# DerrickXuNu/CoBEVT

Hardware: AMD Instinct MI355X
Metric: bev_frames_per_sec (higher is better)
Workload: dtype bf16

## Files before the change

cobevt_amd/csrc/elementwise.hip:

```cpp
#include "warp_common.hpp"
#include "wave_ops.hpp"

namespace cobevt {

template <typename T>
__global__ __launch_bounds__(256) void layernorm_kernel(const T* in, const float* gamma, const float* beta, T* out,
                                                        int rows, int C, float eps, int navg, long avg_stride,
                                                        long in_batch_stride, int rows_per_batch) {
    const int G = C >> 3;
    const int gid = (blockIdx.x * 256 + threadIdx.x) / G;
    const int gl = threadIdx.x & (G - 1);
    if (gid >= rows) return;
    const int bb = gid / rows_per_batch, rr = gid - bb * rows_per_batch;
    const T* src = in + (size_t)bb * in_batch_stride + (size_t)rr * C + gl * 8;
    float v[8];
    load8<T>(src, v);
    if (navg > 1) {
        for (int s = 1; s < navg; ++s) {
            float w[8];
            load8<T>(src + (size_t)s * avg_stride, w);
#pragma unroll
            for (int e = 0; e < 8; ++e) v[e] += w[e];
        }
        const float inv = 1.0f / (float)navg;
#pragma unroll
        for (int e = 0; e < 8; ++e) v[e] *= inv;
    }
    float s = 0.f;
#pragma unroll
    for (int e = 0; e < 8; ++e) s += v[e];
    s = wave_sum_xor(s, G);
    const float mean = s / (float)C;
    float q = 0.f;
#pragma unroll
    for (int e = 0; e < 8; ++e) { const float d = v[e] - mean; q += d * d; }
    q = wave_sum_xor(q, G);
    const float rstd = rsqrtf(q / (float)C + eps);
#pragma unroll
    for (int e = 0; e < 8; ++e) {
        v[e] = (v[e] - mean) * rstd;
        if (gamma) v[e] = v[e] * gamma[gl * 8 + e] + beta[gl * 8 + e];
    }
    store8<T>(out + (size_t)gid * C + gl * 8, v);
}

constexpr int kEmbedPixPerBlock = 256;
constexpr int kRayPixPerBlock = 64;

template <typename T>
__global__ __launch_bounds__(256) void ray_embed_kernel(const float* I_inv, const float* E_inv, const float* plane,
                                                        const float* w_img, const float* w_cam, T* out, int BN,
                                                        int hw, int D) {
    const int G = D >> 3;
    const int gl = threadIdx.x & (G - 1), gp = threadIdx.x / G, ngroups = 256 / G;
    const int bn = blockIdx.y;
    const float* I = I_inv + bn * 9;
    const float* E = E_inv + bn * 16;
    float wi[8][4], ce[8];
#pragma unroll
    for (int e = 0; e < 8; ++e) {
        const int ch = gl * 8 + e;
        const float4 a = *(const float4*)(w_img + ch * 4), c = *(const float4*)(w_cam + ch * 4);
        wi[e][0] = a.x; wi[e][1] = a.y; wi[e][2] = a.z; wi[e][3] = a.w;
        ce[e] = c.x * E[3] + c.y * E[7] + c.z * E[11] + c.w * E[15];
    }
    const int p0 = blockIdx.x * kRayPixPerBlock;
    constexpr int U = 4;
    for (int pb = p0 + gp; pb < min(p0 + kRayPixPerBlock, hw); pb += ngroups * U) {
        float pxs[U], pys[U], pzs[U];
#pragma unroll
        for (int u = 0; u < U; ++u) {
            const int q = min(pb + u * ngroups, hw - 1);
            pxs[u] = plane[q]; pys[u] = plane[hw + q]; pzs[u] = plane[2 * hw + q];
        }
#pragma unroll
        for (int u = 0; u < U; ++u) {
        const int pix = pb + u * ngroups;
        if (pix >= min(p0 + kRayPixPerBlock, hw)) break;
        const float px = pxs[u], py = pys[u], pz = pzs[u];
        float cam[4];
#pragma unroll
        for (int r = 0; r < 3; ++r) cam[r] = I[r * 3 + 0] * px + I[r * 3 + 1] * py + I[r * 3 + 2] * pz;
        cam[3] = 1.f;
        float d4[4];
#pragma unroll
        for (int r = 0; r < 4; ++r)
            d4[r] = E[r * 4 + 0] * cam[0] + E[r * 4 + 1] * cam[1] + E[r * 4 + 2] * cam[2] + E[r * 4 + 3] * cam[3];
        float v[8], ss = 0.f;
#pragma unroll
        for (int e = 0; e < 8; ++e) {
            const float de = wi[e][0] * d4[0] + wi[e][1] * d4[1] + wi[e][2] * d4[2] + wi[e][3] * d4[3];
            v[e] = de - ce[e];
            ss += v[e] * v[e];
        }
        ss = wave_sum_xor(ss, G);
        const float inv = 1.0f / (sqrtf(ss) + 1e-7f);
#pragma unroll
        for (int e = 0; e < 8; ++e) v[e] *= inv;
        store8<T>(out + ((size_t)bn * hw + pix) * D + gl * 8, v);
        }
    }
}

template <typename T>
__global__ __launch_bounds__(256) void bev_embed_kernel(const float* E_inv, const float* world, const float* w_bev,
                                                        const float* b_bev, const float* w_cam, const T* x, T* out,
                                                        int B, int n, int hw, int D, int x_bcast) {
    const int G = D >> 3;
    const int gl = threadIdx.x & (G - 1), gp = threadIdx.x / G, ngroups = 256 / G;
    const int bn = blockIdx.y, b = x_bcast ? 0 : bn / n;
    const float* E = E_inv + bn * 16;
    float wb[8][2], off[8];
#pragma unroll
    for (int e = 0; e < 8; ++e) {
        const int ch = gl * 8 + e;
        const float4 c = *(const float4*)(w_cam + ch * 4);
        wb[e][0] = w_bev[ch * 2 + 0]; wb[e][1] = w_bev[ch * 2 + 1];
        off[e] = c.x * E[3] + c.y * E[7] + c.z * E[11] + c.w * E[15];
    }
    float bb[8];
#pragma unroll
    for (int e = 0; e < 8; ++e) bb[e] = b_bev[gl * 8 + e];
    const int p0 = blockIdx.x * kEmbedPixPerBlock;
    constexpr int U = 4;
    for (int pb = p0 + gp; pb < min(p0 + kEmbedPixPerBlock, hw); pb += ngroups * U) {
        float wxs[U], wys[U], xvs[U][8];
#pragma unroll
        for (int u = 0; u < U; ++u) {
            const int q = min(pb + u * ngroups, hw - 1);
            wxs[u] = world[q]; wys[u] = world[hw + q];
            load8<T>(x + ((size_t)b * hw + q) * D + gl * 8, xvs[u]);
        }
#pragma unroll
        for (int u = 0; u < U; ++u) {
        const int pix = pb + u * ngroups;
        if (pix >= min(p0 + kEmbedPixPerBlock, hw)) break;
        const float wx = wxs[u], wy = wys[u];
        float v[8], ss = 0.f;
#pragma unroll
        for (int e = 0; e < 8; ++e) {
            const float we = wb[e][0] * wx + wb[e][1] * wy + bb[e];
            v[e] = we - off[e];
            ss += v[e] * v[e];
        }
        ss = wave_sum_xor(ss, G);
        const float inv = 1.0f / (sqrtf(ss) + 1e-7f);
#pragma unroll
        for (int e = 0; e < 8; ++e) v[e] = v[e] * inv + xvs[u][e];
        store8<T>(out + ((size_t)bn * hw + pix) * D + gl * 8, v);
        }
    }
}

template <typename T>
__global__ __launch_bounds__(256) void agent_max_kernel(const T* in, T* out, int B, int L, long per8) {
    const long gid = (long)blockIdx.x * 256 + threadIdx.x;
    if (gid >= (long)B * per8) return;
    const long b = gid / per8, i = gid - b * per8;
    float m[8];
    load8<T>(in + ((size_t)b * L * per8 + i) * 8, m);
    for (int l = 1; l < L; ++l) {
        float v[8];
        load8<T>(in + (((size_t)b * L + l) * per8 + i) * 8, v);
#pragma unroll
        for (int e = 0; e < 8; ++e) m[e] = fmaxf(m[e], v[e]);
    }
    store8<T>(out + (size_t)gid * 8, m);
}

template <typename T>
__global__ __launch_bounds__(256) void maxpool3x3s2_kernel(const T* in, T* out, int N, int H, int W, int C, int Ho,
                                                           int Wo) {
    const int G = C >> 3;
    const long gid = ((long)blockIdx.x * 256 + threadIdx.x) / G;
    const int gl = threadIdx.x & (G - 1);
    if (gid >= (long)N * Ho * Wo) return;
    const int n = (int)(gid / (Ho * Wo)), rem = (int)(gid - (long)n * Ho * Wo);
    const int oh = rem / Wo, ow = rem - oh * Wo;
    float m[8];
#pragma unroll
    for (int e = 0; e < 8; ++e) m[e] = -INFINITY;
    for (int kh = 0; kh < 3; ++kh) {
        const int ih = oh * 2 - 1 + kh;
        if (ih < 0 || ih >= H) continue;
        for (int kw = 0; kw < 3; ++kw) {
            const int iw = ow * 2 - 1 + kw;
            if (iw < 0 || iw >= W) continue;
            float v[8];
            load8<T>(in + (((size_t)n * H + ih) * W + iw) * C + gl * 8, v);
#pragma unroll
            for (int e = 0; e < 8; ++e) m[e] = fmaxf(m[e], v[e]);
        }
    }
    store8<T>(out + gid * C + gl * 8, m);
}

template <typename TI, typename TO>
__global__ __launch_bounds__(256) void to_nhwc_kernel(const TI* in, TO* out, int N, int C, int H, int W, long sN, long sC,
                                                      long sH, long sW) {
    const long i = (long)blockIdx.x * 256 + threadIdx.x;
    const long total = (long)N * C * H * W;
    if (i >= total) return;
    const int c = (int)(i % C);
    long r = i / C;
    const int w = (int)(r % W); r /= W;
    const int h = (int)(r % H);
    const int n = (int)(r / H);
    store_elem<TO>(out, i, load_elem<TI>(in, n * sN + c * sC + h * sH + w * sW));
}
template <typename TI, typename TO>
__global__ __launch_bounds__(256) void from_nhwc_kernel(const TI* in, TO* out, int N, int C, int H, int W, long sN,
                                                        long sC, long sH, long sW) {
    const long i = (long)blockIdx.x * 256 + threadIdx.x;
    const long total = (long)N * C * H * W;
    if (i >= total) return;
    const int c = (int)(i % C);
    long r = i / C;
    const int w = (int)(r % W); r /= W;
    const int h = (int)(r % H);
    const int n = (int)(r / H);
    store_elem<TO>(out, n * sN + c * sC + h * sH + w * sW, load_elem<TI>(in, i));
}

template <typename T>
__global__ __launch_bounds__(256) void regroup_kernel(const T* in, const int* record_len, T* out, float* mask, int B,
                                                      int max_cav, long chunks_per_agent) {
    const long i = (long)blockIdx.x * 256 + threadIdx.x;
    const long total = (long)B * max_cav * chunks_per_agent;
    if (i >= total) return;
    const long agent_slot = i / chunks_per_agent, within = i - agent_slot * chunks_per_agent;
    const int b = (int)(agent_slot / max_cav), l = (int)(agent_slot - (long)b * max_cav);
    int off = 0;
    for (int bb = 0; bb < b; ++bb) off += record_len[bb];
    const bool present = l < record_len[b];
    uint4 v = make_uint4(0, 0, 0, 0);
    if (present) v = ((const uint4*)in)[(long)(off + l) * chunks_per_agent + within];
    ((uint4*)out)[i] = v;
    if (within == 0) mask[agent_slot] = present ? 1.f : 0.f;
}

template <typename T>
__global__ __launch_bounds__(256) void sttf_warp_kernel(const T* x, const float* tmat, const float* cav_mask, T* out,
                                                        float* com_mask, const int* record_len, float* cav_out,
                                                        int B, int Lc, int H, int W, int C,
                                                        float discrete_ratio, float downsample_rate) {
    const int G = C >> 3;
    const int bl = blockIdx.y;
    const int b = bl / Lc, l = bl - b * Lc;
    __shared__ Affine th_feat, th_mask;
// ... 315 lines not shown
```

cobevt_amd/csrc/proj_chain128.hip:

```cpp
#include "row_chain.hpp"
#include "wave_ops.hpp"

namespace cobevt {

namespace {

constexpr int kFp = 0, kFn = 32, kMaxNnt = 8;
constexpr int kTab = (kFn + kMaxNnt * 8) * 1024;
constexpr int kSc = 0, kSh = 128, kBp = 256, kBn = 384;
constexpr int kTabFloats = 640;
constexpr int kLdsBytes = kTab + kTabFloats * 4;

template <int NNT, int NW>
__global__ __launch_bounds__(NW * 64, 1) void proj_chain128_kernel(RowChainParams p, int nblk) {
    extern __shared__ __attribute__((aligned(16))) unsigned char smem[];
    const uint4* wl = (const uint4*)smem;
    float* tab = (float*)(smem + kTab);
    const int tid = threadIdx.x, lane = tid & 63, wave = tid >> 6;
    const int h = lane >> 5, ql = lane & 31;

    {
        uint4* dst = (uint4*)smem;
        constexpr int TOTAL = (kFn + NNT * 8) * 64, PER = (TOTAL + NW * 64 - 1) / (NW * 64);
        uint4 tmp[PER];
#pragma unroll
        for (int u = 0; u < PER; ++u) {
            const int i = tid + u * NW * 64, ic = i < TOTAL ? i : TOTAL - 1;
            const int f = ic >> 6, ln = ic & 63, hh = ln >> 5, q = ln & 31;
            const uint4* base = f < kFn ? p.wp + (size_t)f * 64 : p.wn + (size_t)(f - kFn) * 64;
            const unsigned char* a0 = (const unsigned char*)(base + (f < kFn ? ln : q)) + (f < kFn ? 0 : 8 * hh);
            const unsigned char* a1 = f < kFn ? a0 + 8 : (const unsigned char*)(base + 32 + q) + 8 * hh;
            const uint2 lo = *(const uint2*)a0, hi = *(const uint2*)a1;
            tmp[u] = make_uint4(lo.x, lo.y, hi.x, hi.y);
        }
#pragma unroll
        for (int u = 0; u < PER; ++u) {
            const int i = tid + u * NW * 64;
            if (i < TOTAL) dst[i] = tmp[u];
        }
        for (int i = tid; i < kTabFloats; i += NW * 64) {
            float v;
            if (i < kSh) v = p.pre_scale ? p.pre_scale[i] : 1.f;
            else if (i < kBp) v = p.pre_shift ? p.pre_shift[i - kSh] : 0.f;
            else if (i < kBn) v = p.bp ? p.bp[i - kBp] : 0.f;
            else v = (p.bn && i - kBn < p.Nn) ? p.bn[i - kBn] : 0.f;
            tab[i] = v;
        }
    }
    __syncthreads();

    int opq = 0;
    const float relu_floor = (p.pre_scale && p.pre_relu) ? 0.f : -INFINITY;
    auto load_tile = [&](uint4 (&fr)[8], int first) {
#pragma unroll
        for (int g = 0; g < 8; ++g) fr[g] = wl[(first + g) * 64 + lane + opq];
    };
    const int nwaves = gridDim.x * NW;
    for (int blk = blockIdx.x * NW + wave; blk < nblk; blk += nwaves) {
        asm volatile("" : "+v"(opq));
        const int m0 = blk * 32;
        const bool live = m0 + ql < p.M;
        const size_t grow = live ? m0 + ql : p.M - 1;
        const bf16_t* arow = p.a + grow * 128;
        uint4 af[8], sk[8];
#pragma unroll
        for (int g = 0; g < 8; ++g) af[g] = *(const uint4*)(arow + 16 * g + 8 * h);
        if (p.skip) {
            const bf16_t* srow = p.skip + (size_t)(grow % p.skip_rows) * 128;
#pragma unroll
            for (int g = 0; g < 8; ++g) sk[g] = *(const uint4*)(srow + 16 * g + 8 * h);
        } else {
#pragma unroll
            for (int g = 0; g < 8; ++g) sk[g] = make_uint4(0, 0, 0, 0);
        }
#pragma unroll
        for (int g = 0; g < 8; ++g) {
            float v[8];
            chunk_to_f32<bf16_t>(af[g], v);
            const float* sc = tab + kSc + 16 * g + 8 * h + opq;
            const float4 s0 = *(const float4*)sc, s1 = *(const float4*)(sc + 4);
            const float4 t0 = *(const float4*)(sc + (kSh - kSc)), t1 = *(const float4*)(sc + (kSh - kSc) + 4);
            v[0] = fmaxf(fmaf(v[0], s0.x, t0.x), relu_floor); v[1] = fmaxf(fmaf(v[1], s0.y, t0.y), relu_floor);
            v[2] = fmaxf(fmaf(v[2], s0.z, t0.z), relu_floor); v[3] = fmaxf(fmaf(v[3], s0.w, t0.w), relu_floor);
            v[4] = fmaxf(fmaf(v[4], s1.x, t1.x), relu_floor); v[5] = fmaxf(fmaf(v[5], s1.y, t1.y), relu_floor);
            v[6] = fmaxf(fmaf(v[6], s1.z, t1.z), relu_floor); v[7] = fmaxf(fmaf(v[7], s1.w, t1.w), relu_floor);
            af[g] = f32_to_chunk<bf16_t>(v);
        }

        float y[4][16];
        uint4 fr[2][8];
        load_tile(fr[0], kFp);
#pragma unroll
        for (int t = 0; t < 4; ++t) {
            f32x16 acc;
#pragma unroll
            for (int r = 0; r < 16; ++r) acc[r] = 0.f;
            load_tile(fr[(t + 1) & 1], t < 3 ? kFp + (t + 1) * 8 : kFn);
            __builtin_amdgcn_sched_barrier(0);
#pragma unroll
            for (int g = 0; g < 8; ++g) mfma_kgroup<bf16_t>(fr[t & 1][g], af[g], acc);
#pragma unroll
            for (int m = 0; m < 2; ++m) {
                uint2 s0 = make_uint2(sk[2 * t + m].x, sk[2 * t + m].y), s1 = make_uint2(sk[2 * t + m].z, sk[2 * t + m].w);
                half_swap(s0, s1);
                const float4 b0 = *(const float4*)(tab + kBp + 32 * t + 16 * m + 4 * h + opq);
                const float4 b1 = *(const float4*)(tab + kBp + 32 * t + 16 * m + 8 + 4 * h + opq);
                float* d = &y[t][8 * m];
                d[0] = rbf(acc[8 * m + 0] + b0.x + bf2f(s0.x & 0xffff)); d[1] = rbf(acc[8 * m + 1] + b0.y + bf2f(s0.x >> 16));
                d[2] = rbf(acc[8 * m + 2] + b0.z + bf2f(s0.y & 0xffff)); d[3] = rbf(acc[8 * m + 3] + b0.w + bf2f(s0.y >> 16));
                d[4] = rbf(acc[8 * m + 4] + b1.x + bf2f(s1.x & 0xffff)); d[5] = rbf(acc[8 * m + 5] + b1.y + bf2f(s1.x >> 16));
                d[6] = rbf(acc[8 * m + 6] + b1.z + bf2f(s1.y & 0xffff)); d[7] = rbf(acc[8 * m + 7] + b1.w + bf2f(s1.y >> 16));
            }
        }
        if (p.out) {
            bf16_t* orow = p.out + grow * 128;
#pragma unroll
            for (int i = 0; i < 8; ++i) {
                const uint4 pk = pack8(&y[i >> 1][8 * (i & 1)]);
                uint2 r0 = make_uint2(pk.x, pk.y), r1 = make_uint2(pk.z, pk.w);
                half_swap(r0, r1);
                if (live) *(uint4*)(orow + 16 * i + 8 * h) = make_uint4(r0.x, r0.y, r1.x, r1.y);
            }
        }
        if (p.next_ln) {
            float s = 0.f;
#pragma unroll
            for (int t = 0; t < 4; ++t)
#pragma unroll
                for (int r = 0; r < 16; ++r) s += y[t][r];
            const float mean = xhalf_sum(s) * (1.0f / 128.0f);
            float q = 0.f;
#pragma unroll
            for (int t = 0; t < 4; ++t)
#pragma unroll
                for (int r = 0; r < 16; ++r) { const float d = y[t][r] - mean; q += d * d; }
            const float rstd = rsqrtf(xhalf_sum(q) * (1.0f / 128.0f) + p.eps_next);
#pragma unroll
            for (int t = 0; t < 4; ++t)
#pragma unroll
                for (int r = 0; r < 16; ++r) y[t][r] = (y[t][r] - mean) * rstd;
        }
        uint4 yh[8];
#pragma unroll
        for (int t = 0; t < 4; ++t)
#pragma unroll
            for (int u = 0; u < 2; ++u) yh[2 * t + u] = pack8(&y[t][8 * u]);

        bf16_t* nrow = p.out_next + grow * p.Nn;
#pragma unroll
        for (int n = 0; n < NNT; ++n) {
            f32x16 acc;
#pragma unroll
            for (int r = 0; r < 16; ++r) acc[r] = 0.f;
            if (n + 1 < NNT) load_tile(fr[(n + 1) & 1], kFn + (n + 1) * 8);
            __builtin_amdgcn_sched_barrier(0);
#pragma unroll
            for (int g = 0; g < 8; ++g) mfma_kgroup<bf16_t>(fr[n & 1][g], yh[g], acc);
            float nv[16];
#pragma unroll
            for (int k = 0; k < 4; ++k) {
                const float4 b = *(const float4*)(tab + kBn + 32 * n + 8 * k + 4 * h + opq);
                nv[4 * k] = acc[4 * k] + b.x; nv[4 * k + 1] = acc[4 * k + 1] + b.y;
                nv[4 * k + 2] = acc[4 * k + 2] + b.z; nv[4 * k + 3] = acc[4 * k + 3] + b.w;
            }
#pragma unroll
            for (int m = 0; m < 2; ++m) {
                const uint4 pk = pack8(&nv[8 * m]);
                uint2 r0 = make_uint2(pk.x, pk.y), r1 = make_uint2(pk.z, pk.w);
                half_swap(r0, r1);
                if (live) *(uint4*)(nrow + 32 * n + 16 * m + 8 * h) = make_uint4(r0.x, r0.y, r1.x, r1.y);
            }
        }
    }
}

template <int NNT> int launch128(const RowChainParams& p, hipStream_t stream) {
    constexpr int NW = 8;
    cobevt::allow_dynamic_lds<proj_chain128_kernel<NNT, NW>>(kLdsBytes);
    const int nblk = (p.M + 31) / 32;
    int blocks = (nblk + NW - 1) / NW;
    if (blocks > 256) blocks = 256;
    hipLaunchKernelGGL((proj_chain128_kernel<NNT, NW>), dim3((unsigned)blocks), dim3(NW * 64), kLdsBytes, stream, p, nblk);
    return cobevt::launch_status();
}

}

int launch_proj_chain128(const RowChainParams& p, hipStream_t stream) {
    if (p.C != 128 || !p.wn || !p.out_next || p.Nn % 32 != 0 || p.Nn > 32 * kMaxNnt || p.next_act != 0) return -1;
    if (p.M < 32768) return -1;
    switch (p.Nn / 32) {
        case 4: return launch128<4>(p, stream);
        case 8: return launch128<8>(p, stream);
        default: return -1;
    }
}

}
```

cobevt_amd/csrc/row_chain.hip:

```cpp
#include "row_chain.hpp"
#include "wave_ops.hpp"

namespace cobevt {

constexpr int kRcRow = 256 + 16;
constexpr int kRcHRow = 512 + 16;
template <int ROWS> struct RcLds {
    static constexpr int A = 0;
    static constexpr int Y = A + ROWS * kRcRow;
    static constexpr int H = Y + ROWS * kRcRow;
    static constexpr int TOTAL = H + ROWS * kRcHRow;
    static constexpr int BIAS = TOTAL;
    static constexpr int BYTES = TOTAL + 4 * 1536;
};
constexpr int kRcBp = 0, kRcB1 = 128, kRcB2 = 384, kRcPg = 512, kRcPb = 640, kRcBn = 768, kRcBnMax = 768, kRcBiasFloats = 1536;

__device__ __forceinline__ void rc_normalise(float (&v)[16], int sub, int C, float eps) {
    float s = 0.f;
#pragma unroll
    for (int e = 0; e < 16; ++e) s += v[e];
    s = lane8_sum(s);
    const float mean = s / (float)C;
    float q = 0.f;
#pragma unroll
    for (int e = 0; e < 16; ++e) { const float d = (sub * 16 + e) < C ? v[e] - mean : 0.f; q += d * d; }
    q = lane8_sum(q);
    const float rstd = rsqrtf(q / (float)C + eps);
#pragma unroll
    for (int e = 0; e < 16; ++e) v[e] = (sub * 16 + e) < C ? (v[e] - mean) * rstd : 0.f;
}

template <int NPASS, int ROWS, bool FULL, bool MLP = true>
__global__ __launch_bounds__(ROWS * 8, 4) void row_chain_kernel(RowChainParams p) {
    extern __shared__ __attribute__((aligned(16))) unsigned char smem[];
    unsigned char* As = smem + RcLds<ROWS>::A;
    unsigned char* Ys = smem + RcLds<ROWS>::Y;
    unsigned char* Hs = smem + RcLds<ROWS>::H;

    const int tid = threadIdx.x, lane = tid & 63, wave = tid >> 6;
    const int h = lane >> 5, ql = lane & 31;
    const int wm = wave >> 2, wn = wave & 3;
    const int m0 = blockIdx.x * ROWS;
    const int ngc = FULL ? 8 : (p.C * 2 + 31) / 32;
    const int row = wm * 32 + ql;
    const bool row_ok = m0 + row < p.M;

    auto load_frags = [&](uint4 (&b)[8], const uint4* w, int tile, int nkg, int kg0, int n) {
        const uint4* src = w + ((size_t)tile * nkg + kg0) * 64 + lane;
#pragma unroll
        for (int g = 0; g < 8; ++g)
            if (g < n) b[g] = src[g * 64];
        __builtin_amdgcn_sched_barrier(0);
    };
    f32x16 acc;
    auto mma = [&](const unsigned char* A, int a_off, const uint4 (&b)[8], int n, bool zero) {
        if (zero) {
#pragma unroll
            for (int r = 0; r < 16; ++r) acc[r] = 0.f;
        }
#pragma unroll
        for (int g = 0; g < 8; ++g)
            if (g < n) {
                const uint4 af = *(const uint4*)(A + a_off + g * 32);
                mfma_kgroup<bf16_t>(b[g], af, acc);
            }
    };
    const int cbase = wn * 32 + 4 * h;
    const float* sb = (const float*)(smem + RcLds<ROWS>::BIAS);
    {
        float* w = (float*)(smem + RcLds<ROWS>::BIAS);
        constexpr int NT = ROWS * 8, NIT = kRcBiasFloats / NT;
        static_assert(kRcBiasFloats % NT == 0, "bias table fill");
        float val[NIT];
        bool keep[NIT];
#pragma unroll
        for (int it = 0; it < NIT; ++it) {
            const int i = tid + it * NT;
            const float* src = i < kRcB1 ? p.bp : i < kRcB2 ? p.b1 : i < kRcPg ? p.b2 : i < kRcPb ? p.post_g : i < kRcBn ? p.post_b : p.bn;
            const int j = i < kRcB1 ? i : i < kRcB2 ? i - kRcB1 : i < kRcPg ? i - kRcB2 : i < kRcPb ? i - kRcPg : i < kRcBn ? i - kRcPb : i - kRcBn;
            const int n = i < kRcB1 ? p.C : i < kRcB2 ? p.Hd : i < kRcBn ? p.C : p.Nn;
            keep[it] = (src != nullptr) & (j < n);
            val[it] = (src ? src : p.b1)[keep[it] ? j : 0];
        }
#pragma unroll
        for (int it = 0; it < NIT; ++it) w[tid + it * NT] = keep[it] ? val[it] : 0.f;
    }
    auto bias4 = [&](int table, int col0) { return *(const float4*)(sb + table + col0); };
    auto pack4 = [&](float x, float y, float z, float w) { return make_uint2(pack_bf2(x, y), pack_bf2(z, w)); };

    uint4 fa[8], fb[8];
    const int abase = row * kRcRow + h * 16;

    load_frags(fa, p.wp, wn, 8, 0, ngc);
    {
        const int r = tid >> 3, sub = tid & 7;
        const bool ok = m0 + r < p.M;
#pragma unroll
        for (int j = 0; j < 2; ++j) {
            const int k = (sub * 2 + j) * 8;
            uint4 v = make_uint4(0, 0, 0, 0);
            if (ok && k < p.C) v = *(const uint4*)(p.a + (size_t)(m0 + r) * p.C + k);
            if (!MLP && p.pre_scale) {
                float f[8];
                chunk_to_f32<bf16_t>(v, f);
                const float4 s0 = *(const float4*)(p.pre_scale + k), s1 = *(const float4*)(p.pre_scale + k + 4);
                const float4 t0 = *(const float4*)(p.pre_shift + k), t1 = *(const float4*)(p.pre_shift + k + 4);
                const float sc[8] = {s0.x, s0.y, s0.z, s0.w, s1.x, s1.y, s1.z, s1.w}, sh[8] = {t0.x, t0.y, t0.z, t0.w, t1.x, t1.y, t1.z, t1.w};
#pragma unroll
                for (int e = 0; e < 8; ++e) {
                    f[e] = fmaf(f[e], sc[e], sh[e]);
                    if (p.pre_relu) f[e] = fmaxf(f[e], 0.f);
                }
                v = ok ? f32_to_chunk<bf16_t>(f) : make_uint4(0, 0, 0, 0);
            }
            *(uint4*)(As + r * kRcRow + (sub * 2 + j) * 16) = v;
        }
    }
    uint2 skp[4];
#pragma unroll
    for (int k = 0; k < 4; ++k) {
        const int col0 = cbase + 8 * k;
        skp[k] = make_uint2(0, 0);
        if (p.skip && row_ok && col0 < p.C) skp[k] = *(const uint2*)(p.skip + (size_t)((m0 + row) % p.skip_rows) * p.C + col0);
    }
    __syncthreads();

    mma(As, abase, fa, ngc, true);
    if (MLP) load_frags(fb, p.w1, wn, 8, 0, ngc);
    else load_frags(fb, p.wn, wn, 8, 0, ngc);
#pragma unroll
    for (int k = 0; k < 4; ++k) {
        const int col0 = cbase + 8 * k;
        const float4 b = bias4(kRcBp, col0);
        float v0 = acc[4 * k] + b.x + bf2f(skp[k].x & 0xffff), v1 = acc[4 * k + 1] + b.y + bf2f(skp[k].x >> 16);
        float v2 = acc[4 * k + 2] + b.z + bf2f(skp[k].y & 0xffff), v3 = acc[4 * k + 3] + b.w + bf2f(skp[k].y >> 16);
        if (col0 >= p.C) v0 = v1 = v2 = v3 = 0.f;
        *(uint2*)(Ys + row * kRcRow + col0 * 2) = pack4(v0, v1, v2, v3);
    }
    __syncthreads();
    float* stage = (float*)Hs;
    constexpr int SROW = kRcHRow / 4;
    if constexpr (MLP) {

    if (NPASS == 2) load_frags(fa, p.w1, 4 + wn, 8, 0, ngc);
    else load_frags(fa, p.w2, wn, p.Hdp / 16, 0, 8);
    {
        const int r = tid >> 3, sub = tid & 7;
        float v[16];
        chunk_to_f32<bf16_t>(*(const uint4*)(Ys + r * kRcRow + sub * 32), v);
        chunk_to_f32<bf16_t>(*(const uint4*)(Ys + r * kRcRow + sub * 32 + 16), v + 8);
        rc_normalise(v, sub, p.C, p.eps1);
        *(uint4*)(As + r * kRcRow + sub * 32) = f32_to_chunk<bf16_t>(v);
// ... 34 lines not shown
    __syncthreads();
#pragma unroll
    for (int k = 0; k < 4; ++k) {
        const int col0 = cbase + 8 * k;
        const float4 b = bias4(kRcB2, col0);
        const uint2 y = *(const uint2*)(Ys + row * kRcRow + col0 * 2);
        float4 z = make_float4(0.f, 0.f, 0.f, 0.f);
        if (col0 < p.C)
            z = make_float4(acc[4 * k] + b.x + bf2f(y.x & 0xffff), acc[4 * k + 1] + b.y + bf2f(y.x >> 16),
                            acc[4 * k + 2] + b.z + bf2f(y.y & 0xffff), acc[4 * k + 3] + b.w + bf2f(y.y >> 16));
        *(float4*)(stage + row * SROW + col0) = z;
    }
    } else {
#pragma unroll
        for (int k = 0; k < 4; ++k) {
            const int col0 = cbase + 8 * k;
            const uint2 y = *(const uint2*)(Ys + row * kRcRow + col0 * 2);
            *(float4*)(stage + row * SROW + col0) = make_float4(bf2f(y.x & 0xffff), bf2f(y.x >> 16), bf2f(y.y & 0xffff), bf2f(y.y >> 16));
        }
    }
    const int npn = p.wn ? (p.Nn + 127) / 128 : 0;
    __syncthreads();

    {
        const int r = tid >> 3, sub = tid & 7;
        const bool live = m0 + r < p.M;
        float v[16];
#pragma unroll
        for (int e = 0; e < 16; e += 4) {
            const float4 t = *(const float4*)(stage + r * SROW + sub * 16 + e);
            v[e] = t.x; v[e + 1] = t.y; v[e + 2] = t.z; v[e + 3] = t.w;
        }
        if (p.post_g) {
            rc_normalise(v, sub, p.C, p.eps_post);
#pragma unroll
            for (int e = 0; e < 16; e += 4) {
                const float4 g = *(const float4*)(sb + kRcPg + sub * 16 + e), b = *(const float4*)(sb + kRcPb + sub * 16 + e);
                v[e] = v[e] * g.x + b.x; v[e + 1] = v[e + 1] * g.y + b.y;
                v[e + 2] = v[e + 2] * g.z + b.z; v[e + 3] = v[e + 3] * g.w + b.w;
            }
        }
        uint4 o[2];
        o[0] = f32_to_chunk<bf16_t>(v);
        o[1] = f32_to_chunk<bf16_t>(v + 8);
        if (live && (MLP || p.out)) {
#pragma unroll
            for (int j = 0; j < 2; ++j) {
                const int c0 = sub * 16 + j * 8;
                if (c0 < p.C) *(uint4*)(p.out + (size_t)(m0 + r) * p.C + c0) = o[j];
            }
        }
        if (!npn) return;

        if (p.next_ln) {
            chunk_to_f32<bf16_t>(o[0], v);
            chunk_to_f32<bf16_t>(o[1], v + 8);
            rc_normalise(v, sub, p.C, p.eps_next);
            o[0] = f32_to_chunk<bf16_t>(v);
            o[1] = f32_to_chunk<bf16_t>(v + 8);
        }
        *(uint4*)(As + r * kRcRow + sub * 32) = o[0];
        *(uint4*)(As + r * kRcRow + sub * 32 + 16) = o[1];
    }
    __syncthreads();
    auto next_pass = [&](int pass, const uint4 (&cur)[8], uint4 (&nxt)[8]) {
        if (pass + 1 < npn) load_frags(nxt, p.wn, (pass + 1) * 4 + wn, 8, 0, ngc);
        mma(As, abase, cur, ngc, true);
#pragma unroll
        for (int k = 0; k < 4; ++k) {
            const int col0 = pass * 128 + cbase + 8 * k;
            const float4 b = bias4(kRcBn, col0);
            float v0 = acc[4 * k] + b.x, v1 = acc[4 * k + 1] + b.y, v2 = acc[4 * k + 2] + b.z, v3 = acc[4 * k + 3] + b.w;
            if (p.next_act == 1) { v0 = fmaxf(v0, 0.f); v1 = fmaxf(v1, 0.f); v2 = fmaxf(v2, 0.f); v3 = fmaxf(v3, 0.f); }
            else if (p.next_act == 2) { v0 = gelu_bf16(v0); v1 = gelu_bf16(v1); v2 = gelu_bf16(v2); v3 = gelu_bf16(v3); }
            *(uint2*)(Ys + row * kRcRow + (cbase + 8 * k) * 2) = pack4(v0, v1, v2, v3);
        }
        __syncthreads();
        {
            const int r = tid >> 3, sub = tid & 7;
            if (m0 + r < p.M) {
#pragma unroll
                for (int j = 0; j < 2; ++j) {
                    const int c0 = pass * 128 + sub * 16 + j * 8;
                    if (c0 < p.Nn) *(uint4*)(p.out_next + (size_t)(m0 + r) * p.Nn + c0) = *(const uint4*)(Ys + r * kRcRow + sub * 32 + j * 16);
                }
            }
        }
        if (pass + 1 < npn) __syncthreads();
    };
    for (int pass = 0; pass < npn; pass += 2) {
        next_pass(pass, fb, fa);
        if (pass + 1 < npn) next_pass(pass + 1, fa, fb);
    }
}

template <int NPASS, int ROWS, bool FULL, bool MLP = true>
static void launch_chain(const RowChainParams& p, hipStream_t stream) {
    cobevt::allow_dynamic_lds<row_chain_kernel<NPASS, ROWS, FULL, MLP>>(RcLds<ROWS>::BYTES);
    const unsigned blocks = (unsigned)((p.M + ROWS - 1) / ROWS);
    hipLaunchKernelGGL((row_chain_kernel<NPASS, ROWS, FULL, MLP>), dim3(blocks), dim3(ROWS * 8), RcLds<ROWS>::BYTES, stream, p);
}

}

using namespace cobevt;

extern "C" int cobevt_attn_mlp_chain(const void* a, const void* skip, void* out, const void* wp, const float* bp,
                                     const void* w1, const float* b1, const void* w2, const float* b2,
                                     const float* post_gamma, const float* post_beta, const void* wnext, const float* bnext,
                                     void* out_next, const int* dims, float eps1, float eps_post, float eps_next,
                                     hipStream_t stream) {
    if (!a || !out || !wp || !w1 || !b1 || !w2 || !b2 || !dims) return COBEVT_ERR_ARG;
    if (dims[0] != 0 && dims[0] != 1) return COBEVT_ERR_ARG;
    if (dims[0] == 1) {
        if ((post_gamma == nullptr) != (post_beta == nullptr) || (wnext == nullptr) != (out_next == nullptr)) return COBEVT_ERR_ARG;
        const int M = dims[1], sr = dims[9] > 0 ? dims[9] : dims[1];
        if (M < 1 || sr > M || M % sr || (wnext && (dims[7] < 0 || dims[7] > 2))) return COBEVT_ERR_SHAPE;
        const int rc = launch_row_chain_f32(a, skip, out, wp, bp, w1, b1, w2, b2, post_gamma, post_beta, wnext, bnext, out_next, M, dims[2], dims[3],
                                            dims[4], dims[5], dims[6], dims[7], sr, eps1, eps_post, eps_next, stream);
        return rc < 0 ? COBEVT_ERR_UNSUPPORTED : rc;
    }
    RowChainParams p;
    p.a = (const bf16_t*)a; p.skip = (const bf16_t*)skip; p.out = (bf16_t*)out;
    p.wp = (const uint4*)wp; p.bp = bp; p.w1 = (const uint4*)w1; p.b1 = b1; p.w2 = (const uint4*)w2; p.b2 = b2;
    p.post_g = post_gamma; p.post_b = post_beta;
    p.wn = (const uint4*)wnext; p.bn = bnext; p.out_next = (bf16_t*)out_next;
    p.M = dims[1]; p.C = dims[2]; p.Hd = dims[3]; p.Hdp = dims[4];
    p.Nn = dims[5]; p.next_ln = dims[6]; p.next_act = dims[7];
    p.skip_rows = dims[9] > 0 ? dims[9] : p.M;
    p.eps1 = eps1; p.eps_post = eps_post; p.eps_next = eps_next;
    p.pre_scale = p.pre_shift = nullptr; p.pre_relu = 0;
    if (p.M < 1 || p.C < 8 || p.C > 128 || p.C % 8 || p.Hd < 8 || p.Hd > 256 || p.Hd % 8) return COBEVT_ERR_SHAPE;
    if (p.Hdp % 128 || p.Hdp < p.Hd || p.Hdp > 256) return COBEVT_ERR_SHAPE;
    if (p.skip_rows > p.M || p.M % p.skip_rows) return COBEVT_ERR_SHAPE;
    if ((post_gamma == nullptr) != (post_beta == nullptr)) return COBEVT_ERR_ARG;
    if ((wnext == nullptr) != (out_next == nullptr)) return COBEVT_ERR_ARG;
    if (wnext && (p.Nn < 8 || p.Nn % 8 || p.Nn > kRcBnMax || p.next_act < 0 || p.next_act > 2)) return COBEVT_ERR_SHAPE;
    if (dims[8] == 0) {
        const int rc = launch_row_chain64(p, stream);
        if (rc >= 0) return rc;
    }
    const int rows = dims[8] == 64 ? 64 : 32;
    const bool two = p.Hd > 128, full = p.C == 128;
    if (rows == 64) {
        if (two) { if (full) launch_chain<2, 64, true>(p, stream); else launch_chain<2, 64, false>(p, stream); }
        else { if (full) launch_chain<1, 64, true>(p, stream); else launch_chain<1, 64, false>(p, stream); }
    } else {
        if (two) { if (full) launch_chain<2, 32, true>(p, stream); else launch_chain<2, 32, false>(p, stream); }
        else { if (full) launch_chain<1, 32, true>(p, stream); else launch_chain<1, 32, false>(p, stream); }
    }
    return cobevt::launch_status();
}

extern "C" int cobevt_proj_chain(const void* a, const float* pre_scale, const float* pre_shift, const void* skip, const void* wp,
                                 const float* bp, void* out, const void* wnext, const float* bnext, void* out_next, const int* dims,
                                 float eps_next, hipStream_t stream) {
    if (!a || !wp || !wnext || !bnext || !out_next || !dims) return COBEVT_ERR_ARG;
    if ((pre_scale == nullptr) != (pre_shift == nullptr)) return COBEVT_ERR_ARG;
    if (dims[0] != 0) return COBEVT_ERR_UNSUPPORTED;
    RowChainParams p;
    p.a = (const bf16_t*)a; p.skip = (const bf16_t*)skip; p.out = (bf16_t*)out;
    p.wp = (const uint4*)wp; p.bp = bp;
    p.w1 = (const uint4*)wnext; p.b1 = bnext; p.w2 = (const uint4*)wnext; p.b2 = bnext;
    p.post_g = p.post_b = nullptr;
    p.wn = (const uint4*)wnext; p.bn = bnext; p.out_next = (bf16_t*)out_next;
    p.M = dims[1]; p.C = dims[2]; p.Hd = 8; p.Hdp = 128;
    p.Nn = dims[3]; p.next_ln = dims[4]; p.next_act = dims[5];
    p.skip_rows = dims[6] > 0 ? dims[6] : p.M;
    p.pre_scale = pre_scale; p.pre_shift = pre_shift; p.pre_relu = dims[7];
    p.eps1 = 0.f; p.eps_post = 0.f; p.eps_next = eps_next;
    if (p.M < 1 || p.C != 128) return COBEVT_ERR_SHAPE;
    if (p.Nn < 8 || p.Nn % 8 || p.Nn > kRcBnMax || p.next_act < 0 || p.next_act > 2) return COBEVT_ERR_SHAPE;
    if (p.skip_rows > p.M || p.M % p.skip_rows) return COBEVT_ERR_SHAPE;
    if (dims[8] == 0) {
        const int rc = launch_proj_chain128(p, stream);
        if (rc >= 0) return rc;
    }
    launch_chain<1, 32, true, false>(p, stream);
    return cobevt::launch_status();
}
```

cobevt_amd/csrc/row_chain.hpp:

```cpp
#pragma once
#include "common.hpp"

namespace cobevt {

struct RowChainParams {
    const bf16_t* a;
    const bf16_t* skip;
    bf16_t* out;
    const uint4* wp;
    const float* bp;
    const uint4* w1;
    const float* b1;
    const uint4* w2;
    const float* b2;
    const float* post_g;
    const float* post_b;
    const uint4* wn;
    const float* bn;
    bf16_t* out_next;
    int M, C, Hd, Hdp;
    int Nn, next_ln, next_act, skip_rows;
    float eps1, eps_post, eps_next;
    const float* pre_scale;
    const float* pre_shift;
    int pre_relu;
};

int launch_row_chain64(const RowChainParams& p, hipStream_t stream);
int launch_proj_chain128(const RowChainParams& p, hipStream_t stream);

int launch_row_chain_f32(const void* a, const void* skip, void* out, const void* wp, const float* bp, const void* w1, const float* b1,
                         const void* w2, const float* b2, const float* post_g, const float* post_b, const void* wnext, const float* bnext,
                         void* out_next, int M, int C, int Hd, int Hdp, int Nn, int next_ln, int next_act, int skip_rows, float eps1,
                         float eps_post, float eps_next, hipStream_t stream);

}
```

cobevt_amd/host/fax_modules.py:

```python
import torch
import torch.nn as nn

from .. import ops
from ..lib import CobevtHipError
from . import runtime as rt
from . import training
from .runtime import HipModule


def generate_grid(height, width):
    xs = torch.linspace(0, 1, width)
    ys = torch.linspace(0, 1, height)
    gx = xs[None, :].expand(height, width)
    gy = ys[:, None].expand(height, width)
    return torch.stack([gx, gy, torch.ones(height, width)], 0)[None].contiguous()


def get_view_matrix(h=200, w=200, h_meters=100.0, w_meters=100.0, offset=0.0):
    sh = h / h_meters
    sw = w / w_meters
    return [[0., -sw, w / 2.], [-sh, 0., h * offset + h / 2.], [0., 0., 1.]]


class Bottleneck(HipModule):
# ... 72 lines not shown
        self.heads = dim // dim_head
        self.scale = dim_head ** -0.5
        self.window_size = window_size
        self.to_qkv = nn.Linear(dim, dim * 3, bias=False)
        self.attend = nn.Sequential(nn.Softmax(dim=-1), nn.Dropout(dropout))
        self.to_out = nn.Sequential(nn.Linear(dim, dim, bias=False), nn.Dropout(dropout))
        self.rel_pos_bias = nn.Embedding((2 * window_size - 1) ** 2, self.heads)
        pos = torch.arange(window_size)
        gi, gj = torch.meshgrid(pos, pos, indexing="ij")
        grid = torch.stack([gi.reshape(-1), gj.reshape(-1)], -1)
        rel_pos = grid[:, None, :] - grid[None, :, :] + window_size - 1
        rel_pos_indices = (rel_pos * torch.tensor([2 * window_size - 1, 1])).sum(dim=-1)
        self.register_buffer("rel_pos_indices", rel_pos_indices, persistent=False)

    def forward_nhwc(self, x, out=None):
        b, h, w, d = x.shape
        if h != self.window_size or w != self.window_size:
            raise CobevtHipError("FAX global attention expects a %dx%d map" % (self.window_size, self.window_size))
        qkv = ops.linear(x, rt.linear_plan(self, "qkv", self.to_qkv))
        a = torch.empty((b, h, w, d), device=x.device, dtype=x.dtype)
        m = ops.tokmap(0, 1, h, w, h, w)
        table = rt.f32_param(self, "bias", self.rel_pos_bias.weight)
        ops.window_attention(qkv, qkv, qkv, a, m, m, m, b, self.heads, self.scale, 3 * d, 3 * d, 3 * d, d, koff=d,
                             voff=2 * d, bias_table=table, bias_L=1)
        return ops.linear(a, rt.linear_plan(self, "out", self.to_out[0]), out=out)

    def forward(self, x):
        if self.training:
            return training.global_attention(self, x)
        self._require_inference(x)
        return rt.like_input(rt.nchw_view(self.forward_nhwc(rt.to_nhwc(x))), x)


class CrossWinAttention(HipModule):

    def __init__(self, dim, heads, dim_head, qkv_bias, rel_pos_emb=False, norm=nn.LayerNorm):
        super().__init__()
        if dim_head != 32:
            raise CobevtHipError("the HIP attention kernel is built for dim_head = 32")
        self.scale = dim_head ** -0.5
        self.heads = heads
        self.dim_head = dim_head
        self.rel_pos_emb = rel_pos_emb
        self.to_q = nn.Sequential(norm(dim), nn.Linear(dim, heads * dim_head, bias=qkv_bias))
        self.to_k = nn.Sequential(norm(dim), nn.Linear(dim, heads * dim_head, bias=qkv_bias))
        self.to_v = nn.Sequential(norm(dim), nn.Linear(dim, heads * dim_head, bias=qkv_bias))
        self.proj = nn.Linear(heads * dim_head, dim)

    def add_rel_pos_emb(self, x):
        return x

    def _project(self, name, seq, x, out=None):
        return ops.linear(x, rt.linear_plan(self, name, seq[1], ln=seq[0]), out=out)

    def project_kv(self, k_src, v_src, out_k=None, out_v=None):
        return self._project("k", self.to_k, k_src, out_k), self._project("v", self.to_v, v_src, out_v)

    def q_plan(self):
        return rt.linear_plan(self, "q", self.to_q[1], ln=self.to_q[0])

    def attend_projected(self, q_src, kt, vt, qmap, kmap, omap, batch, out_shape, qt=None, ldkv=None, kvoff=0):
        inner = self.heads * self.dim_head
        if qt is None:
            qt = self._project("q", self.to_q, q_src)
        ld = inner if ldkv is None else ldkv
        a = torch.empty(tuple(out_shape) + (inner,), device=qt.device, dtype=qt.dtype)
        ops.window_attention(qt, kt, vt, a, qmap, kmap, omap, batch, self.heads, self.scale, inner, ld, ld, inner,
                             koff=kvoff, voff=kvoff, mean_q=qmap[1] > 1)
        return a

    def attend_core(self, q_src, k_src, v_src, qmap, kmap, omap, batch, out_shape):
        kt, vt = self.project_kv(k_src, v_src)
        return self.attend_projected(q_src, kt, vt, qmap, kmap, omap, batch, out_shape)

    def attend(self, q_src, k_src, v_src, qmap, kmap, omap, batch, skip, out_shape):
        a = self.attend_core(q_src, k_src, v_src, qmap, kmap, omap, batch, out_shape)
        return ops.linear(a, rt.linear_plan(self, "proj", self.proj), residual=skip)

    def forward(self, q, k, v, skip=None):
        if self.training:
            return training.cross_win_attention(self, q, k, v, skip)
        self._require_inference(q, k, v, skip)
        assert k.shape == v.shape
        b, n, X, Y, W1, W2, _ = q.shape
        _, nk, kx, ky, w1, w2, _ = k.shape
        assert X * Y == kx * ky
        qmap = (2, n, X * W1, Y * W2, W1, W2, X, Y)
        kmap = (2, nk, kx * w1, ky * w2, w1, w2, kx, ky)
        omap = (2, 1, X * W1, Y * W2, W1, W2, X, Y)
        sk = rt.as_compute(skip) if skip is not None else None
        z = self.attend(rt.as_compute(q), rt.as_compute(k), rt.as_compute(v), qmap, kmap, omap, b, sk,
                        (b, X, Y, W1, W2))
        return rt.like_input(z, q)


class CrossViewSwapAttention(HipModule):

    def __init__(self, feat_height, feat_width, feat_dim, dim, index, image_height, image_width, qkv_bias, q_win_size,
                 feat_win_size, heads, dim_head, bev_embedding_flag, rel_pos_emb=False, no_image_features=False,
                 skip=True, norm=nn.LayerNorm):
        super().__init__()
        image_plane = generate_grid(feat_height, feat_width)[None]
        image_plane[:, :, 0] *= image_width
        image_plane[:, :, 1] *= image_height
        self.register_buffer("image_plane", image_plane, persistent=False)
        self.feature_linear = nn.Sequential(nn.BatchNorm2d(feat_dim), nn.ReLU(), nn.Conv2d(feat_dim, dim, 1, bias=False))
        if no_image_features:
            self.feature_proj = None
        else:
            self.feature_proj = nn.Sequential(nn.BatchNorm2d(feat_dim), nn.ReLU(), nn.Conv2d(feat_dim, dim, 1, bias=False))
        self.bev_embed_flag = bev_embedding_flag[index]
        if self.bev_embed_flag:
            self.bev_embed = nn.Conv2d(2, dim, 1)
        self.img_embed = nn.Conv2d(4, dim, 1, bias=False)
        self.cam_embed = nn.Conv2d(4, dim, 1, bias=False)
        self.q_win_size = q_win_size[index]
        self.feat_win_size = feat_win_size[index]
        self.rel_pos_emb = rel_pos_emb
        self.cross_win_attend_1 = CrossWinAttention(dim, heads[index], dim_head[index], qkv_bias)
        self.cross_win_attend_2 = CrossWinAttention(dim, heads[index], dim_head[index], qkv_bias)
        self.skip = skip
        self.prenorm_1 = norm(dim)
        self.prenorm_2 = norm(dim)
        self.mlp_1 = nn.Sequential(nn.Linear(dim, 2 * dim), nn.GELU(), nn.Linear(2 * dim, dim))
        self.mlp_2 = nn.Sequential(nn.Linear(dim, 2 * dim), nn.GELU(), nn.Linear(2 * dim, dim))
        self.postnorm = norm(dim)
        self.dim = dim

    def _padded_hw(self, h, w):
        wh, ww = self.feat_win_size
        hp = ((h + wh) // wh) * wh if h % wh != 0 else h
        wp = ((w + ww) // ww) * ww if w % ww != 0 else w
        return hp, wp

    def _proj_mlp(self, name, attn, a, skip, prenorm, mlp, postnorm=None, next_plan=None):
        post = None
        if postnorm is not None:
            post = (rt.f32_param(self, name + ".post.w", postnorm.weight), rt.f32_param(self, name + ".post.b", postnorm.bias),
                    postnorm.eps)
        return ops.attn_mlp_chain(a, skip, rt.linear_plan(attn, "proj", attn.proj),
                                  rt.linear_plan(self, name + ".0", mlp[0], act=2, ln=prenorm),
                                  rt.linear_plan(self, name + ".2", mlp[2]), post, next_plan=next_plan)

    def prepare_kv(self, feature, I_inv, E_inv, batch, out=None):
        bn, h, w, _ = feature.shape
        d, dt = self.dim, feature.dtype
        n = bn // batch
        w1, w2 = self.feat_win_size
        hp, wp = self._padded_hw(h, w)
        padded = (hp, wp) != (h, w)
        plane = rt.f32_param(self, "plane", self.image_plane, (3, h * w))
        w_img = rt.f32_param(self, "w_img", self.img_embed.weight, (d, 4))
        w_cam = rt.f32_param(self, "w_cam", self.cam_embed.weight, (d, 4))
        img = ops.ray_embed(I_inv, E_inv, plane, w_img, w_cam, h * w, d, dt).reshape(bn, h, w, d)

        def kv_buffer(tag):
            if not padded:
                return None
            return self._plan("kvpad.%s.%dx%dx%d" % (tag, bn, hp, wp), [self.img_embed.weight],
                              lambda dt_, dev: torch.zeros((bn, hp, wp, d), device=feature.device, dtype=dt))

        o = out if out is not None else {}
        pk, pv = self._pair_plan("k"), self._pair_plan("v")
        plan_key = rt.conv_plan(self, "fproj", self.feature_proj[2], pre_bn=self.feature_proj[0]) if self.feature_proj is not None else None
        plan_val = rt.conv_plan(self, "flin", self.feature_linear[2], pre_bn=self.feature_linear[0])
        if (not padded and plan_key is not None and ops.proj_chain_fusable(feature, plan_key, pk, img)
                and ops.proj_chain_fusable(feature, plan_val, pv, None)):
            kk = ops.proj_chain(feature, plan_key, pk, residual=img, out_next=o.get("kk"))
            vv = ops.proj_chain(feature, plan_val, pv, out_next=o.get("vv"))
            return {"n": n, "hp": hp, "wp": wp, "kk": kk, "vv": vv}
        if not padded and plan_key is not None and ops.proj_chain_kv_fusable(feature, plan_key, plan_val, pk, pv, img):
            kk, vv = ops.proj_chain_kv(feature, plan_key, plan_val, pk, pv, residual=img, out_k=o.get("kk"), out_v=o.get("vv"))
            return {"n": n, "hp": hp, "wp": wp, "kk": kk, "vv": vv}
        if self.feature_proj is not None:
            key = ops.conv2d(feature, plan_key, residual=img, out=kv_buffer("key"))
        elif padded:
            key = ops.copy_into_interior(img, kv_buffer("key"))
        else:
            key = img
        val = ops.conv2d(feature, plan_val, out=kv_buffer("val"))
        kk = ops.linear(key, pk, out=o.get("kk"))
        vv = ops.linear(val, pv, out=o.get("vv"))
        return {"n": n, "hp": hp, "wp": wp, "kk": kk, "vv": vv}

    def _pair_plan(self, which):
        a1, a2 = getattr(self.cross_win_attend_1, "to_" + which), getattr(self.cross_win_attend_2, "to_" + which)
        if a1[0].eps != a2[0].eps:
            raise CobevtHipError("the two cross attentions normalise their keys / values with different eps")

        def build(dt, dev):
            ws, bs = [], []
            for ln, lin in ((a1[0], a1[1]), (a2[0], a2[1])):
                w = lin.weight.detach().double().cpu()
                b = lin.bias.detach().double().cpu() if lin.bias is not None else torch.zeros(w.shape[0], dtype=torch.float64)
                g, be = ln.weight.detach().double().cpu(), ln.bias.detach().double().cpu()
                bs.append(b + w @ be)
                ws.append(w * g[None, :])
            return ops.ConvPlan(torch.cat(ws), torch.cat(bs), dtype=dt, device=dev, ln_folded_eps=a1[0].eps)
        return self._plan("pair_" + which, rt.module_tensors(a1[0], a1[1], a2[0], a2[1]), build)

    def forward_query(self, index, x, bev, E_inv, kv, next_plan=None):
        b, H, W, d = x.shape
        n, hp, wp = kv["n"], kv["hp"], kv["wp"]
        W1, W2 = self.q_win_size
        w1, w2 = self.feat_win_size
        if self.bev_embed_flag:
            grid = getattr(bev, "grid%d" % index)
            world = rt.f32_param(self, "world%d" % index, grid[:2], (2, H * W))
            w_bev = rt.f32_param(self, "w_bev", self.bev_embed.weight, (d, 2))
            b_bev = rt.f32_param(self, "b_bev", self.bev_embed.bias)
            w_cam = rt.f32_param(self, "w_cam", self.cam_embed.weight, (d, 4))
            q1 = ops.bev_embed_linear(E_inv, world, w_bev, b_bev, w_cam, x.reshape(b, H * W, d), n,
                                      self.cross_win_attend_1.q_plan())
            query, nq = None, n
        else:
            x = x.contiguous()
            query, nq, q1 = x, 1, None
        qmap_n = ops.tokmap(0, nq, H, W, W1, W2)
        qmap_1 = ops.tokmap(0, 1, H, W, W1, W2)
        kwin = ops.tokmap(0, n, hp, wp, w1, w2)
        kgrid = ops.tokmap(1, n, hp, wp, w1, w2)
        if qmap_1[6] * qmap_1[7] != kwin[6] * kwin[7]:
            raise CobevtHipError("query windows %dx%d != key windows %dx%d" % (qmap_1[6], qmap_1[7], kwin[6], kwin[7]))
        inner = self.cross_win_attend_1.heads * self.cross_win_attend_1.dim_head
        a = self.cross_win_attend_1.attend_projected(query, kv["kk"], kv["vv"], qmap_n, kwin, qmap_1, b, (b, H, W), qt=q1,
                                                     ldkv=2 * inner, kvoff=0)
        y, q2 = self._proj_mlp("mlp1", self.cross_win_attend_1, a, x if self.skip else None, self.prenorm_1, self.mlp_1,
                               next_plan=self.cross_win_attend_2.q_plan())
        a = self.cross_win_attend_2.attend_projected(y, kv["kk"], kv["vv"], qmap_1, kgrid, qmap_1, b, (b, H, W), qt=q2,
                                                     ldkv=2 * inner, kvoff=inner)
        return self._proj_mlp("mlp2", self.cross_win_attend_2, a, y if self.skip else None, self.prenorm_2, self.mlp_2,
                              self.postnorm, next_plan=next_plan)

    def forward_nhwc(self, index, x, bev, feature, I_inv, E_inv):
        return self.forward_query(index, x, bev, E_inv, self.prepare_kv(feature, I_inv, E_inv, x.shape[0]))

    def forward(self, index, x, bev, feature, I_inv, E_inv):
        if self.training:
            return training.cross_view_swap_attention(self, index, x, bev, feature, I_inv, E_inv)
        self._require_inference(x, feature, I_inv, E_inv)
        b, n = feature.shape[:2]
        f = rt.to_nhwc(feature.reshape(b * n, *feature.shape[2:]))
        Ii = I_inv.reshape(b * n, 3, 3).to(torch.float32).contiguous()
        Ei = E_inv.reshape(b * n, 4, 4).to(torch.float32).contiguous()
        y = self.forward_nhwc(index, rt.to_nhwc(x), bev, f, Ii, Ei)
        return rt.like_input(rt.nchw_view(y), x)


class _Downsample(HipModule):

    def __init__(self, dim_in, dim_mid, dim_out):
        super().__init__()
        mods = [nn.Conv2d(dim_in, dim_mid, kernel_size=3, stride=1, padding=1, bias=False), nn.PixelUnshuffle(2),
                nn.Conv2d(dim_out, dim_out, 3, padding=1, bias=False), nn.BatchNorm2d(dim_out), nn.ReLU(inplace=True),
                nn.Conv2d(dim_out, dim_out, 1, padding=0, bias=False), nn.BatchNorm2d(dim_out)]
        for i, m in enumerate(mods):
            self.add_module(str(i), m)

    def __getitem__(self, i):
        return getattr(self, str(i))

    def forward_nhwc(self, x, out=None):
        y = ops.conv2d(x, rt.conv_plan(self, "c0", self[0], store_mode=1))
        y = ops.conv2d(y, rt.conv_plan(self, "c2", self[2], self[3], act=1))
        return ops.conv2d(y, rt.conv_plan(self, "c5", self[5], self[6]), out=out)


class FAXModule(HipModule):

    _downsample_div = 4

    def __init__(self, config):
        super().__init__()
        middle = config["middle"]
        dim = config["dim"]
        self.backbone_output_shape = config["backbone_output_shape"]
        assert len(middle) == len(self.backbone_output_shape)
        cross_view = config["cross_view"]
        cross_view_swap = config["cross_view_swap"]
        cross_views, layers, downsample_layers = [], [], []
        for i, (feat_shape, num_layers) in enumerate(zip(self.backbone_output_shape, middle)):
            _, _, _, feat_dim, feat_height, feat_width = tuple(feat_shape)
            cross_views.append(CrossViewSwapAttention(feat_height, feat_width, feat_dim, dim[i], i, **cross_view,
                                                      **cross_view_swap))
            layers.append(nn.Sequential(*[ResNetBottleNeck(dim[i]) for _ in range(num_layers)]))
            if i < len(middle) - 1:
                downsample_layers.append(nn.Sequential(_Downsample(dim[i], dim[i] // self._downsample_div, dim[i + 1])))
        self.bev_embedding = BEVEmbedding(dim[0], **config["bev_embedding"])
        self.cross_views = nn.ModuleList(cross_views)
        self.layers = nn.ModuleList(layers)
        self.downsample_layers = nn.ModuleList(downsample_layers)
        self.self_attn = Attention(dim[-1], **config["self_attn"])

    taps = None

    def forward_features(self, features, I_inv, E_inv, batch, kv=None, levels=None, x=None, out=None):
        nlev = len(self.cross_views)
        first, last = (0, nlev) if levels is None else levels
        if first == 0:
            dt = rt.get_compute_dtype()
            prior = self._plan("prior", [self.bev_embedding.learned_features],
                               lambda d_, dev: self.bev_embedding.learned_features.detach().permute(1, 2, 0).to(dt).contiguous())
            x = prior[None].expand(batch, *prior.shape)
        for i, (cross_view, feature, layer) in enumerate(zip(self.cross_views, features, self.layers)):
            if i < first or i >= last:
                continue
            kvi = kv[i]() if kv is not None else cross_view.prepare_kv(feature, I_inv, E_inv, batch)
            blocks = list(layer)
            y1 = None
            if blocks and not (x.dtype == torch.bfloat16 and ops.USE_BOTTLENECK and x.shape[-1] == 128
                               and blocks[0].conv1.weight.shape[:2] == (32, 128)):
                x, y1 = cross_view.forward_query(i, x, self.bev_embedding, E_inv, kvi, next_plan=blocks[0].entry_plan())
            else:
                x = cross_view.forward_query(i, x, self.bev_embedding, E_inv, kvi)
            for j, blk in enumerate(blocks):
                x = blk.forward_nhwc(x, y1=y1 if j == 0 else None)
            if self.taps is not None:
                self.taps["level%d" % i] = x
# ... 27 lines not shown
```

cobevt_amd/lib.py:

```python
import ctypes
import os

import torch

_HERE = os.path.dirname(os.path.abspath(__file__))
LIB_PATH = os.path.join(_HERE, "csrc", "libcobevt_hip.so")
LIB_PATH = os.environ.get("COBEVT_HIP_LIB") or LIB_PATH

_c_int_p = ctypes.POINTER(ctypes.c_int)
_c_long_p = ctypes.POINTER(ctypes.c_long)
_c_float_p = ctypes.POINTER(ctypes.c_float)
_vp = ctypes.c_void_p

SIGNATURES = {
    "cobevt_abi_version": (ctypes.c_int, []),
    "cobevt_strerror": (ctypes.c_char_p, [ctypes.c_int]),
    "cobevt_conv2d_nhwc": (ctypes.c_int, [_vp, _vp, _vp, _vp, _vp, _vp, _vp, _vp, _c_int_p, _vp]),
    "cobevt_conv3x3_nhwc": (ctypes.c_int, [_vp, _vp, _vp, _vp, _vp, _c_int_p, _vp]),
    "cobevt_basicblock_nhwc": (ctypes.c_int, [_vp, _vp, _vp, _vp, _vp, _vp, _c_int_p, _vp]),
    "cobevt_dsblock_nhwc": (ctypes.c_int, [_vp, _vp, _vp, _vp, _vp, _vp, _vp, _vp, _c_int_p, _vp]),
    "cobevt_conv3x3_wfrag_nhwc": (ctypes.c_int, [_vp, _vp, _vp, _vp, _vp, _c_int_p, _vp]),
    "cobevt_conv3x3_ds_wfrag_nhwc": (ctypes.c_int, [_vp, _vp, _vp, _vp, _vp, _vp, _c_int_p, _vp]),
    "cobevt_stem_conv7x7s2_pool": (ctypes.c_int, [_vp, _vp, _vp, _vp, _c_int_p, _vp]),
    "cobevt_stem_conv7x7s2": (ctypes.c_int, [_vp, _vp, _vp, _vp, _c_int_p, _vp]),
    "cobevt_stem_conv7x7s2_pool_u8": (ctypes.c_int, [_vp, _vp, _vp, _vp, _vp, _c_int_p, _vp]),
    "cobevt_bev_embed_linear_rows": (ctypes.c_int, [_vp] * 9 + [_c_long_p, ctypes.c_float, _vp]),
    "cobevt_linear_rows_wfrag": (ctypes.c_int, [_vp, _vp, _vp, _vp, _vp, _vp, _vp, _c_long_p, ctypes.c_float, _vp]),
    "cobevt_linear_rows": (ctypes.c_int, [_vp, _vp, _vp, _vp, _vp, _vp, _vp, _vp, _vp, _c_long_p, ctypes.c_float, _vp]),
    "cobevt_attn_mlp_chain": (ctypes.c_int, [_vp] * 14 + [_c_int_p, ctypes.c_float, ctypes.c_float, ctypes.c_float, _vp]),
    "cobevt_pairwise_warp": (ctypes.c_int, [_vp] * 5 + [ctypes.c_int] * 6 + [ctypes.c_float, ctypes.c_float, _vp]),
    "cobevt_pairwise_warp_bwd": (ctypes.c_int, [_vp] * 4 + [ctypes.c_int] * 6 + [ctypes.c_float, ctypes.c_float, _vp]),
    "cobevt_agent_message_reduce": (ctypes.c_int, [_vp] * 5 + [ctypes.c_int] * 6 + [_vp]),
    "cobevt_gru_zero_state": (ctypes.c_int, [_vp, _vp, ctypes.c_int, ctypes.c_long, ctypes.c_int, _vp]),
    "cobevt_agent_softmax_sum": (ctypes.c_int, [_vp, ctypes.c_int, _vp, _vp, _vp, _vp] + [ctypes.c_int] * 6 + [_vp]),
    "cobevt_window_attention": (ctypes.c_int, [_vp, _vp, _vp, _vp, _vp, _vp, _c_int_p, ctypes.c_float, _vp]),
    "cobevt_window_attention_ksplit": (ctypes.c_int, [_vp] * 8 + [_c_int_p, ctypes.c_float, ctypes.c_int, ctypes.c_long, _vp]),
    "cobevt_window_attention_lse": (ctypes.c_int, [_vp, _vp, _vp, _vp, _vp, _vp, _vp, _c_int_p, ctypes.c_float, ctypes.c_float,
                                                   ctypes.c_uint, _vp, _vp]),
    "cobevt_conv3x3_head_nchw": (ctypes.c_int, [_vp, _vp, _vp, _vp] + [ctypes.c_int] * 6 + [_vp]),
    "cobevt_weighted_cross_entropy_bwd": (ctypes.c_int, [_vp] * 6 + [ctypes.c_int] * 3 + [_vp]),
    "cobevt_attention_dropout_mask": (ctypes.c_int, [ctypes.c_int] * 5 + [ctypes.c_float, ctypes.c_uint, _vp, _vp]),
    "cobevt_layernorm_bwd": (ctypes.c_int, [_vp] * 6 + [ctypes.c_int, ctypes.c_int, ctypes.c_float, _vp]),
    "cobevt_conv_wgrad": (ctypes.c_int, [_vp, _vp, _vp, _c_int_p, _vp]),
    "cobevt_conv_wgrad_blocked": (ctypes.c_int, [_vp, _vp, _vp, _c_int_p, _vp]),
    "cobevt_gelu": (ctypes.c_int, [_vp, _vp, _vp, ctypes.c_long, _vp]),
    "cobevt_layernorm_fwd_t": (ctypes.c_int, [_vp, _vp, _vp, _vp, ctypes.c_int, ctypes.c_int, ctypes.c_float, _c_int_p, _vp]),
    "cobevt_layernorm_bwd_t": (ctypes.c_int, [_vp] * 6 + [ctypes.c_int, ctypes.c_int, ctypes.c_float, _c_int_p, _vp]),
    "cobevt_gelu_bf16": (ctypes.c_int, [_vp, _vp, _vp, ctypes.c_long, _vp]),
    "cobevt_window_attention_bwd": (ctypes.c_int, [_vp] * 13 + [_c_int_p, ctypes.c_float, ctypes.c_float, ctypes.c_uint, _vp, _vp]),
    "cobevt_layernorm": (ctypes.c_int, [_vp, _vp, _vp, _vp, ctypes.c_int, ctypes.c_int, ctypes.c_int, ctypes.c_float,
                                        ctypes.c_int, ctypes.c_long, ctypes.c_long, ctypes.c_int, _vp]),
    "cobevt_fax_ray_embed": (ctypes.c_int, [_vp, _vp, _vp, _vp, _vp, _vp, ctypes.c_int, ctypes.c_int, ctypes.c_int,
                                            ctypes.c_int, _vp]),
    "cobevt_fax_bev_embed": (ctypes.c_int, [_vp, _vp, _vp, _vp, _vp, _vp, _vp, ctypes.c_int, ctypes.c_int, ctypes.c_int,
                                            ctypes.c_int, ctypes.c_int, ctypes.c_int, _vp]),
    "cobevt_maxpool3x3s2": (ctypes.c_int, [_vp, _vp, ctypes.c_int, ctypes.c_int, ctypes.c_int, ctypes.c_int, ctypes.c_int,
                                           _vp]),
    "cobevt_to_nhwc": (ctypes.c_int, [_vp, ctypes.c_int, _vp, ctypes.c_int, ctypes.c_int, ctypes.c_int, ctypes.c_int,
                                      ctypes.c_int, _c_long_p, _vp]),
    "cobevt_from_nhwc": (ctypes.c_int, [_vp, ctypes.c_int, _vp, ctypes.c_int, ctypes.c_int, ctypes.c_int, ctypes.c_int,
                                        ctypes.c_int, _c_long_p, _vp]),
    "cobevt_regroup": (ctypes.c_int, [_vp, _vp, _vp, _vp, ctypes.c_int, ctypes.c_int, ctypes.c_int, ctypes.c_long, _vp]),
    "cobevt_invert_small": (ctypes.c_int, [_vp, _vp, ctypes.c_int, ctypes.c_int, _vp]),
    "cobevt_resize_nhwc": (ctypes.c_int, [_vp, _vp] + [ctypes.c_int] * 8 + [_vp]),
    "cobevt_channel_affine": (ctypes.c_int, [_vp, _vp, _vp, _vp, ctypes.c_long, ctypes.c_int, ctypes.c_long, _vp]),
    "cobevt_sttf_warp": (ctypes.c_int, [_vp, _vp, _vp, _vp, _vp, _vp, _vp, ctypes.c_int, ctypes.c_int, ctypes.c_int, ctypes.c_int,
                                        ctypes.c_int, ctypes.c_int, ctypes.c_float, ctypes.c_float, _vp]),
    "cobevt_softmax_argmax": (ctypes.c_int, [_vp, _vp, _vp, ctypes.c_int, ctypes.c_int, ctypes.c_int, ctypes.c_int, _vp]),
    "cobevt_seg_class_counts": (ctypes.c_int, [_vp, _vp, _vp, ctypes.c_int, ctypes.c_int, ctypes.c_int, _vp]),
    "cobevt_weighted_cross_entropy": (ctypes.c_int, [_vp, _vp, _vp, _vp, _vp, ctypes.c_int, ctypes.c_int, ctypes.c_int, ctypes.c_int, _vp]),
    "cobevt_linear_rows_small_k": (ctypes.c_int, [_vp, _vp, _vp, _vp, _vp, _vp, _vp, _c_long_p, ctypes.c_float, _vp]),
    "cobevt_bev_embed_linear_rows_small_k": (ctypes.c_int, [_vp] * 9 + [_c_long_p, ctypes.c_float, _vp]),
    "cobevt_sigmoid_focal_loss": (ctypes.c_int, [_vp, _vp, _vp, _vp, _vp, _vp, ctypes.c_int, ctypes.c_int, ctypes.c_int, ctypes.c_int,
                                                 ctypes.c_int, ctypes.c_float, ctypes.c_float, ctypes.c_int, _vp]),
    "cobevt_iou_counts": (ctypes.c_int, [_vp, _vp, _vp, _vp, _vp, _vp, ctypes.c_int, ctypes.c_int, ctypes.c_int, ctypes.c_int,
                                         ctypes.c_int, ctypes.c_int, _vp]),
    "cobevt_agent_max": (ctypes.c_int, [_vp, _vp, ctypes.c_int, ctypes.c_int, ctypes.c_int, ctypes.c_long, _vp]),
    "cobevt_bottleneck_nhwc": (ctypes.c_int, [_vp] * 8 + [_c_int_p, _vp]),
    "cobevt_bottleneck_f32_nhwc": (ctypes.c_int, [_vp] * 9 + [_c_int_p, _vp]),
    "cobevt_attention_index_map": (ctypes.c_int, [_c_int_p, ctypes.c_int, _vp, _vp]),
    "cobevt_attention_bias_index": (ctypes.c_int, [_c_int_p, _c_int_p, ctypes.c_int, _vp, _vp]),
    "cobevt_depthwise_conv_nhwc": (ctypes.c_int, [_vp, _vp, _vp, _vp, _c_int_p, _vp]),
    "cobevt_spatial_mean_nhwc": (ctypes.c_int, [_vp, _vp, ctypes.c_int, ctypes.c_int, ctypes.c_int, ctypes.c_int, _vp]),
    "cobevt_se_gate": (ctypes.c_int, [_vp, _vp, _vp, _vp, _vp, _vp, ctypes.c_int, ctypes.c_int, ctypes.c_int, _vp]),
    "cobevt_mean_linear_rows_small_k": (ctypes.c_int, [_vp, _vp, _vp, _vp, _c_long_p, ctypes.c_float, _vp]),
    "cobevt_proj_chain": (ctypes.c_int, [_vp] * 10 + [_c_int_p, ctypes.c_float, _vp]),
    "cobevt_proj_chain_kv": (ctypes.c_int, [_vp, ctypes.POINTER(ctypes.c_void_p), _c_int_p, ctypes.c_float, _vp]),
    "cobevt_swap_fusion_stage": (ctypes.c_int, [_vp, _vp, _vp, _vp, _c_int_p, _vp, _vp, _vp, _vp, _vp, _vp, _vp, _vp, _vp, _vp, _c_int_p,
                                                ctypes.c_float, ctypes.c_float, ctypes.c_float, _vp]),
    "cobevt_channel_sums": (ctypes.c_int, [_vp, _vp, _vp, _vp, _vp, _vp, ctypes.c_int, ctypes.c_int, ctypes.c_long, ctypes.c_int, _vp]),
    "cobevt_f64_to_f32": (ctypes.c_int, [_vp, _vp, ctypes.c_int, _vp]),
    "cobevt_bn_batch_stats": (ctypes.c_int, [_vp] * 10 + [ctypes.c_int, ctypes.c_int, ctypes.c_long, ctypes.c_int, ctypes.c_float, ctypes.c_float, _vp, _vp]),
    "cobevt_bn_finalize": (ctypes.c_int, [_vp] * 10 + [ctypes.c_int, ctypes.c_long, ctypes.c_float, ctypes.c_float, ctypes.c_int, ctypes.c_int, _vp, _vp]),
    "cobevt_bn_apply": (ctypes.c_int, [_vp, _vp, _vp, _vp, _vp, ctypes.c_int, ctypes.c_long, ctypes.c_int, ctypes.c_int, _vp]),
    "cobevt_bn_backward": (ctypes.c_int, [_vp] * 9 + [ctypes.c_int, _vp, _vp, ctypes.c_int, ctypes.c_long, ctypes.c_int, ctypes.c_int,
                                          ctypes.c_int, _vp]),
    "cobevt_maxpool3x3s2_bwd": (ctypes.c_int, [_vp, _vp, _vp] + [ctypes.c_int] * 5 + [_vp]),
    "cobevt_maxpool3x3s2_bwd_t": (ctypes.c_int, [_vp, _vp, _vp] + [ctypes.c_int] * 5 + [_vp]),
    "cobevt_fax_bev_query_train": (ctypes.c_int, [_vp] * 6 + [_c_int_p, _vp]),
    "cobevt_fax_bev_query_train_bwd": (ctypes.c_int, [_vp] * 9 + [_c_int_p, _vp]),
    "cobevt_group_mean": (ctypes.c_int, [_vp, _vp, ctypes.c_int, ctypes.c_long, ctypes.c_int, ctypes.c_long, ctypes.c_int, _vp]),
    "cobevt_pixel_unshuffle2_nhwc": (ctypes.c_int, [_vp, _vp] + [ctypes.c_int] * 6 + [_vp]),
    "cobevt_upsample_nearest2_nhwc": (ctypes.c_int, [_vp, _vp] + [ctypes.c_int] * 6 + [_vp]),
    "cobevt_sttf_warp_bwd": (ctypes.c_int, [_vp, _vp, _vp, _vp] + [ctypes.c_int] * 5 + [ctypes.c_float, ctypes.c_float, _vp]),
    "cobevt_conv_weight_rows": (ctypes.c_int, [_vp, _vp, _vp, _c_int_p, _vp]),
    "cobevt_conv3_weight_operands": (ctypes.c_int, [_vp, _vp, _vp, _c_int_p, _vp]),
    "cobevt_conv3_weight_operands2": (ctypes.c_int, [_vp, ctypes.POINTER(ctypes.c_void_p), _c_int_p, _vp]),
    "cobevt_linear_weight_frags": (ctypes.c_int, [_vp, _vp, _vp, _c_int_p, _vp]),
    "cobevt_conv_wgrad3_chunks": (ctypes.c_int, [_c_int_p]),
    "cobevt_conv_wgrad3": (ctypes.c_int, [_vp, _vp, _vp, _vp, _c_int_p, _vp]),
    "cobevt_linear_wgrad_chunks": (ctypes.c_int, [_c_long_p]),
    "cobevt_linear_wgrad": (ctypes.c_int, [_vp, _vp, _vp, _vp, _c_long_p, _vp]),
    "cobevt_wgrad_block_operand": (ctypes.c_int, [_vp, _vp, _c_int_p, _vp]),
    "cobevt_swish": (ctypes.c_int, [_vp, _vp, _vp, ctypes.c_int, ctypes.c_long, _vp]),
    "cobevt_depthwise_wgrad": (ctypes.c_int, [_vp, _vp, _vp, _c_int_p, _vp]),
    "cobevt_resize_bilinear_bwd": (ctypes.c_int, [_vp, _vp] + [ctypes.c_int] * 7 + [_vp]),
    "cobevt_sigmoid_focal_loss_bwd": (ctypes.c_int, [_vp] * 7 + [ctypes.c_int] * 5 + [ctypes.c_float, ctypes.c_float, ctypes.c_int, _vp]),
    "cobevt_peer_window_alloc": (ctypes.c_int, [ctypes.c_long, ctypes.POINTER(_vp), _vp]),
    "cobevt_peer_window_open": (ctypes.c_int, [_vp, ctypes.POINTER(_vp)]),
    "cobevt_peer_window_close": (ctypes.c_int, [_vp]),
    "cobevt_peer_window_free": (ctypes.c_int, [_vp]),
    "cobevt_peer_window_status": (ctypes.c_int, [_vp, ctypes.c_long, _c_int_p, _c_int_p, _vp]),
    "cobevt_peer_window_status_async": (ctypes.c_int, [_vp, ctypes.c_long, _vp, _vp]),
    "cobevt_calibrate_mfma": (ctypes.c_int, [_vp, _vp, ctypes.c_int, ctypes.c_int, _vp]),
    "cobevt_calibrate_copy": (ctypes.c_int, [_vp, _vp, ctypes.c_long, _vp]),
    "cobevt_calibrate_clock_khz": (ctypes.c_int, [_c_int_p, _c_int_p]),
    "cobevt_peer_exchange": (ctypes.c_int, [_vp, ctypes.POINTER(_vp), ctypes.c_int, ctypes.c_int, ctypes.c_int, ctypes.c_long,
                                            _c_int_p, _c_int_p, ctypes.c_long, ctypes.c_long, _vp]),
    "cobevt_host_fetch": (ctypes.c_int, [_vp, _vp, ctypes.c_long, ctypes.c_int, _vp]),
    "cobevt_channel_gate_nhwc": (ctypes.c_int, [_vp, _vp, _vp, ctypes.c_int, ctypes.c_int, ctypes.c_int, ctypes.c_int, _vp]),
    "cobevt_pillar_vfe": (ctypes.c_int, [_vp] * 8 + [_c_int_p, _c_float_p, _vp]),
    "cobevt_scatter_rows": (ctypes.c_int, [_vp, _vp, _vp, ctypes.c_int, ctypes.c_long] + [ctypes.c_int] * 4 + [_vp]),
    "cobevt_pillar_train_scratch": (ctypes.c_int, [ctypes.c_long, _c_long_p, _c_long_p]),
    "cobevt_pillar_train_stats": (ctypes.c_int, [_vp] * 17 + [_c_int_p, _c_float_p, ctypes.c_int, ctypes.c_float, ctypes.c_float, _vp]),
    "cobevt_pillar_train_bwd": (ctypes.c_int, [_vp] * 16 + [_c_int_p, _c_float_p, ctypes.c_int, _vp]),
    "cobevt_gather_rows": (ctypes.c_int, [_vp, _vp, _vp, ctypes.c_int, ctypes.c_long] + [ctypes.c_int] * 4 + [_vp]),
    "cobevt_voxelize_scratch": (ctypes.c_int, [_c_long_p, _c_long_p]),
    "cobevt_voxelize_points": (ctypes.c_int, [_vp] * 7 + [_c_long_p, _c_float_p, _vp]),
    "cobevt_detect_scratch": (ctypes.c_int, [ctypes.c_long, _c_long_p]),
    "cobevt_detect_post": (ctypes.c_int, [ctypes.POINTER(_vp)] * 3 + [_vp, _c_int_p, ctypes.c_int, ctypes.c_int, ctypes.c_float,
                                          ctypes.c_float] + [_vp] * 5 + [_vp]),
    "cobevt_nms_rotated": (ctypes.c_int, [_vp, _vp, ctypes.c_long, ctypes.c_int, ctypes.c_float] + [_vp] * 5 + [_vp]),
    "cobevt_delta_to_boxes3d": (ctypes.c_int, [_vp, _vp, _vp] + [ctypes.c_int] * 4 + [_vp]),
    "cobevt_rotated_iou": (ctypes.c_int, [_vp, _vp, _vp, ctypes.c_long, ctypes.c_long, _vp]),
}

_libs = {}
_variant = ""
_encoder_variant = None
_encoder_depth = 0
VARIANTS = ("", "f32s", "f32h")
LIB_PATH_F32S = os.environ.get("COBEVT_HIP_LIB_F32S") or os.path.join(_HERE, "csrc", "libcobevt_hip_f32s.so")
LIB_PATH_F32H = os.environ.get("COBEVT_HIP_LIB_F32H") or os.path.join(_HERE, "csrc", "libcobevt_hip_f32h.so")


class CobevtHipError(RuntimeError):
    pass


def set_variant(variant):
    global _variant
    if variant not in VARIANTS:
        raise CobevtHipError("unknown library variant %r" % (variant,))
    _variant = variant


def get_variant():
    return _encoder_variant if (_encoder_depth > 0 and _encoder_variant is not None) else _variant


def set_encoder_variant(variant):
    global _encoder_variant
    if variant is not None and variant not in VARIANTS:
        raise CobevtHipError("unknown library variant %r" % (variant,))
    _encoder_variant = variant


def get_encoder_variant():
    return _encoder_variant


class encoder_scope(object):

    def __enter__(self):
        global _encoder_depth
        _encoder_depth += 1
        return self

    def __exit__(self, *exc):
        global _encoder_depth
        _encoder_depth -= 1
        return False


def load(variant=None):
    v = get_variant() if variant is None else variant
    lib = _libs.get(v)
    if lib is not None:
        return lib
    path = {"f32s": LIB_PATH_F32S, "f32h": LIB_PATH_F32H}.get(v, LIB_PATH)
    if not os.path.exists(path):
        raise CobevtHipError(
            "%s not found at %s — build it with `python -m cobevt_amd.build` "
            "(there is no CPU / eager fallback for the hot path)" % (os.path.basename(path), path))
    lib = ctypes.CDLL(path)
    for name, (res, args) in SIGNATURES.items():
        fn = getattr(lib, name)
        fn.restype = res
        fn.argtypes = args
    if lib.cobevt_abi_version() != 1:
        raise CobevtHipError("%s ABI version mismatch" % os.path.basename(path))
    _libs[v] = lib
    return lib


def check(rc, what):
    if rc != 0:
        msg = load().cobevt_strerror(rc).decode()
        raise CobevtHipError("%s failed: %s (code %d)" % (what, msg, rc))


def call(name, *args, variant=None):
    check(getattr(load(variant), name)(*args), name)
```

cobevt_amd/ops.py:

```python
import ctypes
import os
import math
from collections import namedtuple

import numpy as np
import torch

from . import lib as _L
from .lib import CobevtHipError

BF16, FP32 = 0, 1
USE_CONV3X3 = True
USE_CONV3_S2 = True
USE_CONV3_SMALL_TILES = True
USE_CONV3_DS = True
USE_CONV3_WFRAG = True
CONV3_VARIANT = 0
USE_GEMM_ROWS = True
USE_GEMM_ROWS2 = False
USE_GEMM_ROWS3 = True
GEMM_ROWS3_MIN_M = 0
GEMM_ROWS3_MAX_K = 512
GEMM_ROWS3_STRIDED = 1
GEMM_ROWS3_ROWS64_MIN_M = 0
USE_STEM_POOL = True
USE_STEM = True
ROW_CHAIN_ROWS = 0
USE_ROW_CHAIN = True
USE_BOTTLENECK_F32 = True
USE_GEMM_ROWS3_F32 = True
USE_ROW_CHAIN_F32 = True
BASICBLOCK_TILE_ROWS = 0
USE_BASICBLOCK = True
BASICBLOCK_MAX_C = 128
USE_DSBLOCK = True
USE_EMBED_GEMM = False
USE_EMBED_GEMM3 = True
USE_CHAIN_NEXT = True
USE_HEAD_CONV = True
USE_PROJ_CHAIN = True
USE_PROJ_CHAIN_KV = True
USE_PROJ_CHAIN_WAVE = True
USE_SWAP_STAGE = True
USE_BOTTLENECK = True
ATTN_VARIANT = 0
USE_ATTN_BIG_RESIDENT = False
ATTN_KSPLIT = 2
ATTN_QSPLIT = 0

INT_KNOBS = ("CONV3_VARIANT", "BASICBLOCK_TILE_ROWS", "ROW_CHAIN_ROWS", "GEMM_ROWS3_MIN_M", "GEMM_ROWS3_MAX_K", "GEMM_ROWS3_STRIDED",
             "GEMM_ROWS3_ROWS64_MIN_M", "BASICBLOCK_MAX_C", "ATTN_VARIANT", "ATTN_QSPLIT", "ATTN_KSPLIT")


def dcode(dtype):
    if dtype == torch.bfloat16:
        return BF16
    if dtype == torch.float32:
        return FP32
    raise CobevtHipError("compute dtype must be torch.bfloat16 or torch.float32, got %s" % dtype)


def _apply_env_flags():
    for item in os.environ.get("COBEVT_FLAGS", "").split(","):
        if "=" in item:
            k, v = item.split("=", 1)
            k = k.strip()
            if k not in globals() or not (k.startswith("USE_") or k in INT_KNOBS):
                raise CobevtHipError("COBEVT_FLAGS: unknown switch %r" % k)
            globals()[k] = int(v) if not k.startswith("USE_") else bool(int(v))


_apply_env_flags()


def _p(t):
    return None if t is None else ctypes.c_void_p(t.data_ptr())


def _stream():
    return ctypes.c_void_p(torch.cuda.current_stream().cuda_stream)


def _need_cuda(*ts):
    for t in ts:
        if t is not None and not t.is_cuda:
            raise CobevtHipError("cobevt_amd kernels need tensors on a ROCm device (got a CPU tensor); "
                                 "there is no CPU fallback")


def _ints(vals):
    return (ctypes.c_int * len(vals))(*[int(v) for v in vals])


_PROFILE = None


class LaunchProfile(object):

    def __init__(self):
        self.records = []

    def __enter__(self):
        global _PROFILE
        _PROFILE = self
        return self

    def __exit__(self, *exc):
        global _PROFILE
        _PROFILE = None

    def summary(self, by_shape=False):
        torch.cuda.synchronize()
        out = {}
        for fam, flops, nbytes, e0, e1 in self.records:
            if not by_shape:
                fam = fam.split("|")[0]
            d = out.setdefault(fam, {"calls": 0, "ms": 0.0, "flops": 0.0, "bytes": 0.0})
            d["calls"] += 1
            d["ms"] += e0.elapsed_time(e1)
            d["flops"] += flops
            d["bytes"] += nbytes
        return out


class _Timed(object):
    __slots__ = ("fam", "flops", "nbytes", "e0")

    def __init__(self, fam, flops, nbytes):
        self.fam, self.flops, self.nbytes = fam, flops, nbytes

    def __enter__(self):
        self.e0 = torch.cuda.Event(enable_timing=True)
        self.e0.record()

    def __exit__(self, *exc):
        e1 = torch.cuda.Event(enable_timing=True)
        e1.record()
        _PROFILE.records.append((self.fam, self.flops, self.nbytes, self.e0, e1))


class _NoTime(object):
    def __enter__(self):
        pass

    def __exit__(self, *exc):
        pass


_NOTIME = _NoTime()


def _timed(fam, flops_fn):
    if _PROFILE is None:
        return _NOTIME
    f, b = flops_fn()
    return _Timed(fam, f, b)


def bn_affine(bn):
    g = bn.weight.detach().double() if bn.weight is not None else torch.ones_like(bn.running_var).double()
    b = bn.bias.detach().double() if bn.bias is not None else torch.zeros_like(bn.running_var).double()
    s = g / torch.sqrt(bn.running_var.detach().double() + bn.eps)
    return s, b - bn.running_mean.detach().double() * s


class ConvPlan(object):

    def __init__(self, weight, bias=None, bn=None, pre_bn=None, pre_relu=False, stride=1, pad=0, act=0,
                 upsample=False, store_mode=0, dtype=torch.bfloat16, device="cuda", smallc=False, ln=None,
                 ln_folded_eps=None, pad_br=None):
        w = weight.detach().double().cpu()
        if w.dim() == 2:
            w = w[:, :, None, None]
        cout, cin, kh, kw = w.shape
        asym = pad_br is not None and int(pad_br) != int(pad)
        self.pad_br = int(pad if pad_br is None else pad_br)
        b = bias.detach().double().cpu() if bias is not None else torch.zeros(cout, dtype=torch.float64)
        has_bias = bias is not None or bn is not None
        self.has_ln, self.ln_eps = False, 0.0
        if ln_folded_eps is not None:
            if ln is not None or kh != 1 or kw != 1 or bn is not None or pre_bn is not None:
                raise CobevtHipError("ln_folded_eps applies to plain Linear / 1x1 layers without another ln")
            self.has_ln, self.ln_eps = True, float(ln_folded_eps)
        if ln is not None:
            if kh != 1 or kw != 1 or bn is not None or pre_bn is not None:
                raise CobevtHipError("LayerNorm folding applies to plain Linear / 1x1 layers")
            g, be = ln.weight.detach().double().cpu(), ln.bias.detach().double().cpu()
            b = b + (w[:, :, 0, 0] @ be)
            w = w * g[None, :, None, None]
            has_bias = True
            self.has_ln, self.ln_eps = True, float(ln.eps)
        if bn is not None:
            s, sh = bn_affine(bn)
            s, sh = s.cpu(), sh.cpu()
            w = w * s[:, None, None, None]
            b = b * s + sh
        self.dtype = dtype
        self.code = dcode(dtype)
        bke = 32 if self.code == BF16 else 16
        ch = 8 if self.code == BF16 else 4
        K = kh * kw * cin
        kpad = (K + bke - 1) // bke * bke
        wk = torch.zeros(cout, kpad, dtype=torch.float64)
        wk[:, :K] = w.permute(0, 2, 3, 1).reshape(cout, K)
# ... 413 lines not shown
        _L.call("cobevt_bottleneck_f32_nhwc", _p(x), _p(y1), _p(p1.wfrag_rows), _p(p1.bias), _p(p2.wfrag), _p(p2.bias), _p(p3.wfrag_rows),
                _p(p3.bias), _p(out), dims, _stream())
    return out


def linear(x, plan, residual=None, out=None):
    lead = x.shape[:-1]
    rows = int(math.prod(lead)) if len(lead) else 1
    x4 = x.reshape(1, 1, rows, x.shape[-1])
    r4 = residual.reshape(1, 1, rows, plan.cout) if residual is not None else None
    o4 = None
    if out is not None:
        if tuple(out.shape) != tuple(lead) + (plan.cout,) or not out.is_contiguous() or out.dtype != x.dtype:
            raise CobevtHipError("linear: `out` must be a contiguous %s tensor of dtype %s" % (tuple(lead) + (plan.cout,), x.dtype))
        o4 = out.reshape(1, 1, rows, plan.cout)
    y = conv2d(x4, plan, residual=r4, out=o4)
    return out if out is not None else y.reshape(*lead, plan.cout)


def layernorm(x, gamma, beta, eps=1e-5, out=None):
    _need_cuda(x, gamma, beta)
    if not x.is_contiguous():
        raise CobevtHipError("layernorm: input must be contiguous")
    c = x.shape[-1]
    rows = x.numel() // c
    if out is None:
        out = torch.empty_like(x)
    _L.call("cobevt_layernorm", _p(x), _p(gamma), _p(beta), _p(out), dcode(x.dtype), rows, c, float(eps), 1, 0, 0, 0, _stream())
    return out


def mean_layernorm(x, gamma, beta, eps=1e-5):
    _need_cuda(x, gamma, beta)
    b, l, r, c = x.shape
    if not x.is_contiguous():
        raise CobevtHipError("mean_layernorm: input must be contiguous")
    out = torch.empty((b, r, c), device=x.device, dtype=x.dtype)
    _L.call("cobevt_layernorm", _p(x), _p(gamma), _p(beta), _p(out), dcode(x.dtype), b * r, c, float(eps), l, r * c, l * r * c, r,
            _stream())
    return out


def mean_ln_linear(x, plan):
    _need_cuda(x)
    b, l, r, c = x.shape
    if not (USE_GEMM_ROWS3 and x.dtype == torch.bfloat16 and x.is_contiguous() and plan.wfrag_rows is not None and plan.kp_rows == 128
            and plan.K == c and c % 8 == 0 and plan.cout % 8 == 0 and plan.cout <= 4096 and l <= 64 and plan.pre_scale is None
            and plan.stride == 1):
        return None
    out = torch.empty((b, r, plan.cout), device=x.device, dtype=x.dtype)
    dims = (ctypes.c_long * 8)(0, b, l, r, c, plan.cout, int(plan.has_ln), plan.act)

    def cost():
        return 2.0 * b * r * c * plan.cout, float((b * l * r * c + b * r * plan.cout + c * plan.cout) * 2)

    with _timed("gemm_rows|mean%d %d->%d M=%d ln" % (l, c, plan.cout, b * r), cost):
        _L.call("cobevt_mean_linear_rows_small_k", _p(x), _p(plan.wfrag_rows), _p(plan.bias), _p(out), dims, ctypes.c_float(plan.ln_eps),
                _stream())
    return out


def tokmap(mode, ncam, hh, ww, w1, w2):
    if hh % w1 or ww % w2:
        raise CobevtHipError("map %dx%d not divisible by window %dx%d" % (hh, ww, w1, w2))
    return (int(mode), int(ncam), int(hh), int(ww), int(w1), int(w2), hh // w1, ww // w2)


def window_attention(q, k, v, out, qmap, kmap, omap, batch, heads, scale, ldq, ldk, ldv, ldo, qoff=0, koff=0, voff=0,
                     ooff=0, bias_table=None, bias_L=1, mask=None, mean_q=False, variant=None, qsplit=None, ksplit=None):
    _need_cuda(q, k, v, out, bias_table, mask)
    code = dcode(q.dtype) | ((ATTN_VARIANT if variant is None else int(variant)) << 8) | \
        ((ATTN_QSPLIT if qsplit is None else int(qsplit)) << 16)
    if k.dtype != q.dtype or v.dtype != q.dtype or out.dtype != q.dtype:
        raise CobevtHipError("window_attention: q/k/v/out dtypes differ")
    L = qmap[6] * qmap[7]
    dims = _ints([code, batch, L, heads, ldq, ldk, ldv, ldo, qoff, koff, voff, ooff,
                  0 if bias_table is None else 1, 0 if bias_table is None else bias_table.shape[0], bias_L,
                  int(mean_q)] + list(qmap) + list(kmap) + list(omap))
    def cost():
        nq = qmap[1] * qmap[4] * qmap[5]
        nk = kmap[1] * kmap[4] * kmap[5]
        esz = q.element_size()
        d = heads * 32
        nbytes = batch * L * (nq + 2 * nk + nq // (qmap[1] if mean_q else 1)) * d * esz
        pairs = nq * nk // (qmap[1] if int(mean_q) == 2 else 1)
        return 4.0 * batch * L * heads * pairs * 32, float(nbytes)

    nq_, nk_ = qmap[1] * qmap[4] * qmap[5], kmap[1] * kmap[4] * kmap[5]
    ks = ATTN_KSPLIT if ksplit is None else int(ksplit)
    big_resident = (USE_ATTN_BIG_RESIDENT and ksplit is None and q.dtype == torch.bfloat16 and bias_table is None and mask is None and not mean_q
                    and 512 < nk_ <= 1024 and (ATTN_VARIANT if variant is None else int(variant)) == 0 and omap[1] == qmap[1])
    use_ks = (ks > 1 and not big_resident and not mean_q and nk_ >= 1024 and batch * L * heads * ((nq_ + 127) // 128) * ks <= 1024
              and out.is_contiguous() and ldo == out.shape[-1] and ooff == 0 and omap[1] == qmap[1])
    if int(mean_q) == 2:
        use_ks = ksplit is not None and ks > 1
        if use_ks and not (out.is_contiguous() and ldo == out.shape[-1] and ooff == 0):
            raise CobevtHipError("window_attention: the camera-paired key split writes a contiguous `out` (ldo = width, ooff = 0)")
    with _L.encoder_scope(), _timed("attention|B%d L%d h%d Nq%d Nk%d%s" % (batch, L, heads, nq_, nk_, " ks%d" % ks if use_ks else ""), cost):
        if use_ks:
            rows = out.numel() // out.shape[-1]
            part_out = torch.empty((ks, rows, heads * 32), device=out.device, dtype=out.dtype)
            part_lse = torch.empty((ks, rows, heads), device=out.device, dtype=torch.float32)
            _L.call("cobevt_window_attention_ksplit", _p(q), _p(k), _p(v), _p(out), _p(bias_table), _p(mask), _p(part_out), _p(part_lse),
                    dims, ctypes.c_float(scale), ks, rows, _stream())
        else:
            _L.call("cobevt_window_attention", _p(q), _p(k), _p(v), _p(out), _p(bias_table), _p(mask), dims, ctypes.c_float(scale),
                    _stream())
    return out


PAIRED_KSPLIT_MAX = 16
PAIRED_KSPLIT_WG = 512


def paired_ksplit(batch, heads, qmap, kmap):
    L = qmap[6] * qmap[7]
    wg = batch * L * heads * ((qmap[4] * qmap[5] + 127) // 128)
    tiles = kmap[1] * ((kmap[4] * kmap[5] + 63) // 64)
    ks = min(PAIRED_KSPLIT_MAX, tiles, PAIRED_KSPLIT_WG // wg)
    return ks if ks >= 2 else None


def attention_index_map(tmap, batch, device):
    L, ntok = tmap[6] * tmap[7], tmap[1] * tmap[4] * tmap[5]
    rows = torch.empty((batch, L, ntok), device=device, dtype=torch.int32)
    _need_cuda(rows)
    _L.call("cobevt_attention_index_map", _ints(tmap), batch, _p(rows), _stream())
    return rows


def attention_bias_index(qmap, kmap, bias_L, device):
    nq, nk = qmap[1] * qmap[4] * qmap[5], kmap[1] * kmap[4] * kmap[5]
    idx = torch.empty((nq, nk), device=device, dtype=torch.int32)
    _need_cuda(idx)
    _L.call("cobevt_attention_bias_index", _ints(qmap), _ints(kmap), int(bias_L), _p(idx), _stream())
    return idx


def agent_max(x):
    _need_cuda(x)
    if not x.is_contiguous():
        raise CobevtHipError("agent_max: input must be contiguous")
    b, l = x.shape[:2]
    out = torch.empty((b,) + tuple(x.shape[2:]), device=x.device, dtype=x.dtype)
    per = out[0].numel()
    _L.call("cobevt_agent_max", _p(x), _p(out), dcode(x.dtype), b, l, per, _stream())
    return out


def ray_embed(i_inv, e_inv, image_plane, w_img, w_cam, hw, dim, dtype):
    _need_cuda(i_inv, e_inv, image_plane, w_img, w_cam)
    bn = i_inv.shape[0]
    out = torch.empty((bn, hw, dim), device=i_inv.device, dtype=dtype)
    _L.call("cobevt_fax_ray_embed", _p(i_inv), _p(e_inv), _p(image_plane), _p(w_img), _p(w_cam), _p(out), dcode(dtype), bn, hw, dim,
            _stream())
    return out


def batch_broadcast(x):
    return x.dim() >= 2 and x.shape[0] > 1 and x.stride(0) == 0 and x[0].is_contiguous()


def bev_embed(e_inv, world, w_bev, b_bev, w_cam, x, n):
    _need_cuda(e_inv, world, w_bev, b_bev, w_cam, x)
    b, hw, d = x.shape
    bcast = batch_broadcast(x)
    if not bcast:
        x = x.contiguous()
    out = torch.empty((b, n, hw, d), device=x.device, dtype=x.dtype)
    _L.call("cobevt_fax_bev_embed", _p(e_inv), _p(world), _p(w_bev), _p(b_bev), _p(w_cam), _p(x), _p(out), dcode(x.dtype), b, n, hw, d,
            int(bcast), _stream())
    return out


def bev_embed_linear(e_inv, world, w_bev, b_bev, w_cam, x, n, plan):
    b, hw, d = x.shape
    bcast = batch_broadcast(x)
    wave_level = d == 128 and plan.cout == 128 and b * n <= 32
    fused3 = ((USE_EMBED_GEMM3 == 2 or (USE_EMBED_GEMM3 and wave_level)) and USE_GEMM_ROWS3 and plan.code == BF16 and plan.has_ln
              and plan.K == d and d <= 128 and d % 8 == 0
              and plan.kp_rows == 128 and plan.wfrag_rows is not None and hw % 32 == 0 and plan.stride == 1
              and plan.pre_scale is None and plan.act == 0 and plan.cout % 8 == 0 and (bcast or x.is_contiguous()))
    if fused3:
        _need_cuda(e_inv, world, w_bev, b_bev, w_cam, x)
        out = torch.empty((b, n, hw, plan.cout), device=x.device, dtype=x.dtype)
        dims = (ctypes.c_long * 8)(plan.code, b, n, hw, d, plan.cout, 1, int(bcast))

        def cost3():
            m = b * n * hw
            return 2.0 * m * plan.cout * d, float((hw if bcast else x.numel() // d) * d * 2 + plan.cout * d * 2 + out.numel() * 2)

        with _timed("gemm_rows|embed %d->%d M=%d ln r32" % (d, plan.cout, b * n * hw), cost3):
            _L.call("cobevt_bev_embed_linear_rows_small_k", _p(e_inv), _p(world), _p(w_bev), _p(b_bev), _p(w_cam), _p(x),
                    _p(plan.wfrag_rows), _p(plan.bias), _p(out), dims, ctypes.c_float(plan.ln_eps), _stream())
        return out
    fused = (USE_EMBED_GEMM and USE_GEMM_ROWS and plan.has_ln and ln_fusable(plan) and plan.K == d and hw % 128 == 0
             and plan.stride == 1 and plan.pre_scale is None and plan.act == 0 and x.is_contiguous())
    if not fused:
        return linear(bev_embed(e_inv, world, w_bev, b_bev, w_cam, x, n), plan)
    _need_cuda(e_inv, world, w_bev, b_bev, w_cam, x)
    out = torch.empty((b, n, hw, plan.cout), device=x.device, dtype=x.dtype)
    dims = (ctypes.c_long * 8)(plan.code, b, n, hw, d, plan.cout, plan.kp_rows, 1)

    def cost():
        m = b * n * hw
        esz = 2 if plan.code == BF16 else 4
        return 2.0 * m * plan.cout * d, float(x.numel() * esz + plan.cout * d * esz + out.numel() * esz)

    with _timed("gemm_rows|embed %d->%d M=%d ln" % (d, plan.cout, b * n * hw), cost):
        _L.call("cobevt_bev_embed_linear_rows", _p(e_inv), _p(world), _p(w_bev), _p(b_bev), _p(w_cam), _p(x), _p(plan.wgt_rows),
                _p(plan.bias), _p(out), dims, ctypes.c_float(plan.ln_eps), _stream())
    return out


def stem_pool(x, plan):
    _need_cuda(x)
    n, h, w, cin = x.shape
    fused = (USE_STEM_POOL and USE_STEM and plan.wgt_stem is not None and plan.cout == 64 and plan.act == 1
             and h % 4 == 0 and w % 4 == 0 and x.dtype == torch.float32 and x.is_contiguous())
    if not fused:
        return maxpool3x3s2(conv2d(x, plan))
    out = torch.empty((n, h // 4, w // 4, 64), device=x.device, dtype=plan.dtype)
    dims = _ints([plan.code, n, h, w])

    def cost():
        esz = 2 if plan.code == BF16 else 4
        return 2.0 * n * (h // 2) * (w // 2) * 64 * 147, float(x.numel() * 4 + out.numel() * esz)

    with _timed("stem7x7|pool %dx%dx%d" % (n, h, w), cost):
        _L.call("cobevt_stem_conv7x7s2_pool", _p(x), _p(plan.wgt_stem), _p(plan.bias), _p(out), dims, _stream())
    return out


def stem_pool_u8(x, lut, plan):
    _need_cuda(x, lut)
    n, h, w, cin = x.shape
    if not (plan.wgt_stem is not None and plan.cout == 64 and plan.act == 1 and h % 4 == 0 and w % 4 == 0 and cin == 3
            and x.dtype == torch.uint8 and x.is_contiguous() and lut.dtype == torch.float32 and tuple(lut.shape) == (3, 256)
            and lut.is_contiguous()):
        raise CobevtHipError("stem_pool_u8: needs contiguous uint8 frames (N, H, W, 3) with H, W multiples of 4, a (3, 256) fp32 table "
                             "and the ResNet stem plan; got %s %s" % (tuple(x.shape), x.dtype))
    out = torch.empty((n, h // 4, w // 4, 64), device=x.device, dtype=plan.dtype)
    dims = _ints([plan.code, n, h, w])

    def cost():
        esz = 2 if plan.code == BF16 else 4
        return 2.0 * n * (h // 2) * (w // 2) * 64 * 147, float(x.numel() + out.numel() * esz)

    with _timed("stem7x7|pool u8 %dx%dx%d" % (n, h, w), cost):
        _L.call("cobevt_stem_conv7x7s2_pool_u8", _p(x), _p(lut), _p(plan.wgt_stem), _p(plan.bias), _p(out), dims, _stream())
    return out


def host_fetch(src_pinned, dst, blocks=0):
    _need_cuda(dst)
    if src_pinned.is_cuda or not src_pinned.is_pinned():
        raise CobevtHipError("host_fetch: the source must be a pinned host tensor (tensor.pin_memory())")
    nbytes = dst.numel() * dst.element_size()
    if (tuple(src_pinned.shape) != tuple(dst.shape) or src_pinned.dtype != dst.dtype or not src_pinned.is_contiguous() or not dst.is_contiguous()
            or nbytes % 16):
        raise CobevtHipError("host_fetch: contiguous tensors of one shape / dtype, a multiple of 16 bytes")
    _L.call("cobevt_host_fetch", ctypes.c_void_p(src_pinned.data_ptr()), _p(dst), nbytes, int(blocks), _stream())
    return dst


def maxpool3x3s2(x):
    _need_cuda(x)
    n, h, w, c = x.shape
    ho, wo = (h + 2 - 3) // 2 + 1, (w + 2 - 3) // 2 + 1
    out = torch.empty((n, ho, wo, c), device=x.device, dtype=x.dtype)
    _L.call("cobevt_maxpool3x3s2", _p(x), _p(out), dcode(x.dtype), n, h, w, c, _stream())
    return out


def to_nhwc(x, dtype):
    _need_cuda(x)
    n, c, h, w = x.shape
    v = x.permute(0, 2, 3, 1)
    if x.dtype == dtype and v.is_contiguous():
        return v
    out = torch.empty((n, h, w, c), device=x.device, dtype=dtype)
    strides = (ctypes.c_long * 4)(*x.stride())
    _L.call("cobevt_to_nhwc", _p(x), dcode(x.dtype), _p(out), dcode(dtype), n, c, h, w, strides, _stream())
    return out


def from_nhwc(x, dtype):
    _need_cuda(x)
    n, h, w, c = x.shape
    out = torch.empty((n, c, h, w), device=x.device, dtype=dtype)
    strides = (ctypes.c_long * 4)(*out.stride())
    _L.call("cobevt_from_nhwc", _p(x), dcode(x.dtype), _p(out), dcode(dtype), n, c, h, w, strides, _stream())
    return out


def copy_into_interior(x, dst):
    _need_cuda(x, dst)
    n, h, w, c = x.shape
    if dst.dtype != x.dtype or not x.is_contiguous() or not dst.is_contiguous() or dst.shape[0] != n or dst.shape[3] != c \
            or dst.shape[1] < h or dst.shape[2] < w:
        raise CobevtHipError("copy_into_interior: dst must be a contiguous (N, >= h, >= w, C) map of x's dtype")
    sN, sH, sW, sC = dst.stride()
    strides = (ctypes.c_long * 4)(sN, sC, sH, sW)
    _L.call("cobevt_from_nhwc", _p(x), dcode(x.dtype), _p(dst), dcode(dst.dtype), n, c, h, w, strides, _stream())
    return dst


def regroup(x, record_len, max_cav):
# ... 311 lines not shown
    return ob, osc, oi, oc


def sttf_warp(x, tmat, cav_mask, discrete_ratio, downsample_rate, want_mask=True, record_len=None, max_cav=None):
    _need_cuda(x, tmat, cav_mask, record_len)
    if tmat.dtype != torch.float32 or not tmat.is_contiguous() or not x.is_contiguous():
        raise CobevtHipError("sttf_warp: tmat must be contiguous fp32, x contiguous")
    if record_len is not None:
        if record_len.dtype != torch.int32 or x.dim() != 4:
            raise CobevtHipError("sttf_warp: record_len must be int32 on the device and x (N, H, W, C)")
        b, l = record_len.shape[0], int(max_cav)
        _, h, w, c = x.shape
        out = torch.empty((b, l, h, w, c), device=x.device, dtype=x.dtype)
        cav = torch.empty((b, l), device=x.device, dtype=torch.float32)
    else:
        b, l, h, w, c = x.shape
        out = torch.empty_like(x)
        cav = None
    if tuple(tmat.shape[:2]) != (b, l):
        raise CobevtHipError("sttf_warp: tmat must be (B, L, 4, 4)")
    com = torch.empty((b, h, w, 1, l), device=x.device, dtype=torch.float32) if want_mask else None
    _L.call("cobevt_sttf_warp", _p(x), _p(tmat), _p(cav_mask), _p(out), _p(com), _p(record_len), _p(cav), dcode(x.dtype), b, l, h, w, c,
            ctypes.c_float(discrete_ratio), ctypes.c_float(downsample_rate), _stream())
    return (out, com, cav) if record_len is not None else (out, com)


def pairwise_warp(x, pairwise, record_len, max_cav, discrete_ratio, downsample_rate):
    _need_cuda(x, pairwise, record_len)
    if record_len.dtype != torch.int32 or x.dim() != 4 or pairwise.dtype != torch.float32:
        raise CobevtHipError("pairwise_warp: record_len int32 on the device, x (N, H, W, C), pairwise fp32")
    b, l = record_len.shape[0], int(max_cav)
    _, h, w, c = x.shape
    if tuple(pairwise.shape) != (b, l, l, 4, 4):
        raise CobevtHipError("pairwise_warp: pairwise must be (B, max_cav, max_cav, 4, 4)")
    nb = torch.empty((b, l, l, h, w, c), device=x.device, dtype=x.dtype)
    roi = torch.empty((b, l, l, h, w), device=x.device, dtype=torch.float32)
    _L.call("cobevt_pairwise_warp", _p(x), _p(pairwise.contiguous()), _p(record_len), _p(nb), _p(roi), dcode(x.dtype), b, l, h, w, c,
            ctypes.c_float(discrete_ratio), ctypes.c_float(downsample_rate), _stream())
    return nb, roi


def agent_message_reduce(msg, ego, roi, record_len, mode):
    _need_cuda(msg, ego, roi, record_len)
    b, l, _, h, w, c = msg.shape
    out = torch.zeros_like(ego)
    _L.call("cobevt_agent_message_reduce", _p(msg), _p(ego), _p(roi), _p(record_len), _p(out), dcode(msg.dtype), b, l, h * w, c,
            {"avg": 0, "max": 1}[mode], _stream())
    return out


def gru_zero_state(x):
    _need_cuda(x)
    c = x.shape[-1] // 2
    out = torch.empty(x.shape[:-1] + (c,), device=x.device, dtype=x.dtype)
    _L.call("cobevt_gru_zero_state", _p(x), _p(out), dcode(x.dtype), x.numel() // (2 * c), c, _stream())
    return out


def agent_softmax_sum(score, nb, roi, record_len, n_agents, use_mask=True):
    _need_cuda(score, nb, roi, record_len)
    b, l, _, h, w, c = nb.shape
    out = torch.zeros((n_agents, h, w, c), device=nb.device, dtype=nb.dtype)
    _L.call("cobevt_agent_softmax_sum", _p(score), score.shape[-1], _p(nb), _p(roi), _p(record_len), _p(out), dcode(nb.dtype), b, l, h * w,
            c, int(bool(use_mask)), _stream())
    return out


def invert_small(m):
    _need_cuda(m)
    d = m.shape[-1]
    x = m.to(torch.float32).contiguous()
    out = torch.empty_like(x)
    _L.call("cobevt_invert_small", _p(x), _p(out), x.numel() // (d * d), d, _stream())
    return out


def resize_nhwc(x, ho, wo, mode):
    _need_cuda(x)
    n, h, w, c = x.shape
    out = torch.empty((n, ho, wo, c), device=x.device, dtype=x.dtype)
    _L.call("cobevt_resize_nhwc", _p(x), _p(out), dcode(x.dtype), n, h, w, c, ho, wo, 0 if mode == "nearest" else 1, _stream())
    return out


def channel_affine(x, scale, shift):
    _need_cuda(x, scale, shift)
    if x.dtype != torch.float32 or not x.is_contiguous():
        x = x.to(torch.float32).contiguous()
    out = torch.empty_like(x)
    n, c = x.shape[0], x.shape[1]
    _L.call("cobevt_channel_affine", _p(x), _p(scale), _p(shift), _p(out), n, c, x.numel() // (n * c), _stream())
    return out


def chain_next_fusable(plan_n, c):
    return (plan_n is not None and plan_n.wfrag_rows is not None and plan_n.stride == 1 and plan_n.kp_rows == 128 and plan_n.K == c
            and plan_n.cout % 8 == 0 and plan_n.cout <= 768 and plan_n.pre_scale is None and not plan_n.pre_relu
            and plan_n.act <= 2)


def attn_mlp_chain(a, skip, plan_p, plan_1, plan_2, post_ln=None, next_plan=None):
    _need_cuda(a, skip)
    c, hd = plan_p.cout, plan_1.cout
    skip_rows = 0
    if skip is not None and batch_broadcast(skip) and skip.shape == a.shape:
        skip_rows = skip[0].numel() // c
    f32 = a.dtype == torch.float32
    fusable = (USE_ROW_CHAIN and (a.dtype == torch.bfloat16 or (f32 and USE_ROW_CHAIN_F32 and c == 128 and hd == 256 and plan_2.kp_rows == 256))
               and plan_p.wfrag_rows is not None and plan_1.wfrag_rows is not None
               and plan_2.wfrag_rows is not None and plan_2.kp_rows <= 256 and plan_1.has_ln and plan_1.act == 2 and plan_p.act == 0
               and plan_2.act == 0 and not plan_p.has_ln and not plan_2.has_ln and plan_p.K == c and plan_1.K == c
               and plan_2.K == hd and plan_2.cout == c and c <= 128 and c % 8 == 0 and hd <= 256 and hd % 8 == 0
               and plan_p.kp_rows == 128 and plan_1.kp_rows == 128 and a.shape[-1] == c and a.is_contiguous()
               and (skip is None or skip.dtype == a.dtype)
               and (skip is None or skip_rows or (skip.is_contiguous() and skip.shape == a.shape)))
    if not fusable:
        y = linear(a, plan_p, residual=skip.contiguous() if skip is not None else None)
        z = linear(linear(y, plan_1), plan_2, residual=y)
        z = layernorm(z, post_ln[0], post_ln[1], post_ln[2]) if post_ln is not None else z
        return (z, linear(z, next_plan)) if next_plan is not None else z
    m = a.numel() // c
    out = torch.empty_like(a)
    fuse_next = USE_CHAIN_NEXT and chain_next_fusable(next_plan, c)
    nn_ = next_plan.cout if fuse_next else 0
    out_next = torch.empty(a.shape[:-1] + (nn_,), device=a.device, dtype=a.dtype) if fuse_next else None
    dims = _ints([plan_p.code, m, c, hd, plan_2.kp_rows, nn_, int(next_plan.has_ln) if fuse_next else 0,
                  next_plan.act if fuse_next else 0, ROW_CHAIN_ROWS, skip_rows])
    pg, pb, pe = post_ln if post_ln is not None else (None, None, 0.0)

    def cost():
        flops = 2.0 * m * (c * c + 2 * c * hd + c * nn_)
        esz = a.element_size()
        return flops, float((2 * m + (0 if skip is None else skip_rows or m)) * c * esz + m * nn_ * esz + (c * c + 2 * c * hd + c * nn_) * esz)

    with _timed("row_chain|C%d H%d M=%d%s%s" % (c, hd, m, " post" if post_ln is not None else "",
                                                  " +next%d" % nn_ if fuse_next else ""), cost):
        _L.call("cobevt_attn_mlp_chain", _p(a), _p(skip), _p(out), _p(plan_p.wfrag_rows), _p(plan_p.bias), _p(plan_1.wfrag_rows),
                _p(plan_1.bias), _p(plan_2.wfrag_rows), _p(plan_2.bias), _p(pg), _p(pb), _p(next_plan.wfrag_rows) if fuse_next else None,
                _p(next_plan.bias) if fuse_next else None, _p(out_next), dims, ctypes.c_float(plan_1.ln_eps), ctypes.c_float(pe),
                ctypes.c_float(next_plan.ln_eps if fuse_next else 0.0), _stream())
    if next_plan is None:
        return out
    return out, (out_next if fuse_next else linear(out, next_plan))


def proj_chain_fusable(x, plan_p, next_plan, residual):
    c = x.shape[-1]
    return (USE_PROJ_CHAIN and x.dtype == torch.bfloat16 and c == 128 and x.is_contiguous() and plan_p.wfrag_rows is not None
            and plan_p.kp_rows == 128 and plan_p.K == c and plan_p.cout == c and plan_p.act == 0 and not plan_p.has_ln
            and plan_p.stride == 1 and chain_next_fusable(next_plan, c)
            and (residual is None or (residual.is_contiguous() and residual.shape == x.shape and residual.dtype == x.dtype)))


def proj_chain(x, plan_p, next_plan, residual=None, out_next=None):
    _need_cuda(x, residual)
    c, nn_ = 128, next_plan.cout
    m = x.numel() // c
    if out_next is None:
        out_next = torch.empty(x.shape[:-1] + (nn_,), device=x.device, dtype=x.dtype)
    elif out_next.numel() != m * nn_ or not out_next.is_contiguous() or out_next.dtype != x.dtype:
        raise CobevtHipError("proj_chain: `out_next` must be a contiguous (.., %d) buffer of dtype %s" % (nn_, x.dtype))
    dims = _ints([0, m, c, nn_, int(next_plan.has_ln), next_plan.act, 0, plan_p.pre_relu, 0 if USE_PROJ_CHAIN_WAVE else 1])

    def cost():
        return 2.0 * m * (c * c + c * nn_), float(m * (c * (2 if residual is not None else 1) + nn_) * 2 + (c * c + c * nn_) * 2)

    with _timed("row_chain|proj C%d M=%d +next%d" % (c, m, nn_), cost):
        _L.call("cobevt_proj_chain", _p(x), _p(plan_p.pre_scale), _p(plan_p.pre_shift), _p(residual), _p(plan_p.wfrag_rows),
                _p(plan_p.bias), None, _p(next_plan.wfrag_rows), _p(next_plan.bias), _p(out_next), dims, ctypes.c_float(next_plan.ln_eps),
                _stream())
    return out_next


def proj_chain_kv_fusable(x, plan_key, plan_val, next_key, next_val, residual):
    k = x.shape[-1]
    if not (USE_PROJ_CHAIN_KV and x.dtype == torch.bfloat16 and x.is_contiguous() and k in (256, 384, 512)):
        return False
    for pl in (plan_key, plan_val):
        if pl is None:
            continue
        if not (pl.wfrag_rows is not None and pl.kp_rows == k and pl.K == k and pl.cout == 128 and pl.act == 0 and not pl.has_ln
                and pl.stride == 1):
            return False
    for pn in (next_key, next_val):
        if not (chain_next_fusable(pn, 128) and pn.act == 0):
            return False
    return (plan_val is not None and next_key.cout == next_val.cout and next_key.has_ln == next_val.has_ln and next_key.ln_eps == next_val.ln_eps
            and (residual is None or (plan_key is not None and residual.is_contiguous() and residual.dtype == x.dtype
                                      and tuple(residual.shape) == tuple(x.shape[:-1]) + (128,))))


def proj_chain_kv(x, plan_key, plan_val, next_key, next_val, residual=None, out_k=None, out_v=None):
    _need_cuda(x, residual)
    k, nn_ = x.shape[-1], next_key.cout
    m = x.numel() // k
    outs = []
    for o in (out_k, out_v):
        if o is None:
            o = torch.empty(x.shape[:-1] + (nn_,), device=x.device, dtype=x.dtype)
        elif o.numel() != m * nn_ or not o.is_contiguous() or o.dtype != x.dtype:
            raise CobevtHipError("proj_chain_kv: result buffers must be contiguous (.., %d) of dtype %s" % (nn_, x.dtype))
        outs.append(o)
    ptrs = (ctypes.c_void_p * 18)()
    for s_, (pp, pn, res, o) in enumerate(((plan_key, next_key, residual, outs[0]), (plan_val, next_val, None, outs[1]))):
        vals = (pp.pre_scale, pp.pre_shift, pp.wfrag_rows, pp.bias, res, pn.wfrag_rows, pn.bias, None, o)
        for j, t in enumerate(vals):
            ptrs[9 * s_ + j] = None if t is None else t.data_ptr()
    dims = _ints([0, m, k, nn_, int(next_key.has_ln), 2, plan_key.pre_relu, 0, plan_val.pre_relu, 0])

    def cost():
        return 2.0 * 2 * m * (k * 128 + 128 * nn_), float(m * (k + (128 if residual is not None else 0) + 2 * nn_) * 2 + 2 * (k * 128 + 128 * nn_) * 2)

    with _timed("row_chain|proj kv K%d M=%d +next%d" % (k, m, nn_), cost):
        _L.call("cobevt_proj_chain_kv", _p(x), ptrs, dims, ctypes.c_float(next_key.ln_eps), _stream())
    return outs[0], outs[1]


def swap_stage_fusable(qkv, x, tmap, heads, plan_p, plan_1, plan_2, next_plan, mask):
    c = x.shape[-1]
    nk = tmap[1] * tmap[4] * tmap[5]
    return (USE_SWAP_STAGE and x.dtype == torch.bfloat16 and qkv.dtype == torch.bfloat16 and c == 128 and heads == 4
            and tmap[0] in (0, 1) and nk <= 384 and x.is_contiguous() and qkv.is_contiguous() and qkv.shape[-1] == 3 * c
            and plan_p.wfrag_rows is not None and plan_1.wfrag_rows is not None and plan_2.wfrag_rows is not None
            and plan_p.kp_rows == 128 and plan_1.kp_rows == 128 and plan_2.kp_rows in (128, 256) and plan_1.has_ln
            and plan_1.act == 2 and plan_p.act == 0 and plan_2.act == 0 and not plan_p.has_ln and not plan_2.has_ln
            and plan_p.K == c and plan_1.K == c and plan_2.K == plan_1.cout and plan_2.cout == c and plan_1.cout % 8 == 0
            and plan_1.cout <= 256 and plan_p.cout == c
            and (next_plan is None or (chain_next_fusable(next_plan, c) and next_plan.cout <= 384 and next_plan.has_ln
                                       and next_plan.act == 0))
            and (mask is None or (mask.dtype == torch.float32 and mask.is_contiguous())))


SWAP_STAGE_BIAS_FLOATS = 10240


def swap_stage(qkv, x, tmap, batch, heads, scale, bias_table, bias_L, mask, plan_p, plan_1, plan_2, next_plan=None):
    _need_cuda(qkv, x, bias_table, mask)
    c, hd = 128, plan_1.cout
    out = torch.empty_like(x)
    nn_ = next_plan.cout if next_plan is not None else 0
    qkv_next = torch.empty(x.shape[:-1] + (nn_,), device=x.device, dtype=x.dtype) if next_plan is not None else None
    bias_rows = (2 * bias_L - 1) * (2 * tmap[4] - 1) * (2 * tmap[5] - 1)
    if bias_table.numel() != SWAP_STAGE_BIAS_FLOATS or bias_table.dtype != torch.float32 or not bias_table.is_contiguous():
        raise CobevtHipError("swap_stage: bias table must be the flat fp32 image of stage_bias_table()")
    dims = _ints([0, batch, c, heads, hd, plan_2.kp_rows, nn_, bias_rows, bias_L])
    m = x.numel() // c
    nk = tmap[1] * tmap[4] * tmap[5]

    def cost():
        flops = 4.0 * m * nk * c + 2.0 * m * (c * c + 2 * c * hd + c * nn_)
        return flops, float(m * (3 * c + 2 * c + nn_) * 2 + (c * c + 2 * c * hd + c * nn_) * 2)

    with _timed("swap_stage|mode%d M=%d Nk%d H%d%s" % (tmap[0], m, nk, hd, " +next%d" % nn_ if nn_ else ""), cost):
        _L.call("cobevt_swap_fusion_stage", _p(qkv), _p(x), _p(out), _p(qkv_next), _ints(tmap), _p(bias_table), _p(mask),
                _p(plan_p.wfrag_rows), _p(plan_p.bias), _p(plan_1.wfrag_rows), _p(plan_1.bias), _p(plan_2.wfrag_rows), _p(plan_2.bias),
                _p(next_plan.wfrag_rows) if next_plan is not None else None, _p(next_plan.bias) if next_plan is not None else None, dims,
                ctypes.c_float(scale), ctypes.c_float(plan_1.ln_eps), ctypes.c_float(next_plan.ln_eps if next_plan is not None else 0.0),
                _stream())
    return out, qkv_next


def softmax_argmax(seg_logits):
    _need_cuda(seg_logits)
    if seg_logits.dim() != 4:
        raise CobevtHipError("softmax_argmax expects (N, C, H, W) logits, got %s" % (tuple(seg_logits.shape),))
    x = seg_logits.contiguous()
    n, c, h, w = x.shape
    prob = torch.empty((n, c, h, w), device=x.device, dtype=torch.float32)
    seg_map = torch.empty((n, h, w), device=x.device, dtype=torch.int64)
    _L.call("cobevt_softmax_argmax", _p(x), _p(prob), _p(seg_map), dcode(x.dtype), n, c, h * w, _stream())
    return prob, seg_map


def seg_class_counts(pred, gt, num_classes):
    _need_cuda(pred, gt)
    if pred.shape != gt.shape or pred.dim() != 3:
        raise CobevtHipError("seg_class_counts expects two (N, H, W) maps, got %s and %s" % (tuple(pred.shape), tuple(gt.shape)))
    p64, g64 = pred.to(torch.int64).contiguous(), gt.to(torch.int64).contiguous()
    n, h, w = p64.shape
    counts = torch.empty((n, num_classes + 1, 3), device=pred.device, dtype=torch.int64)
    _L.call("cobevt_seg_class_counts", _p(p64), _p(g64), _p(counts), n, h * w, num_classes, _stream())
    host = counts.cpu()
    if int(host[:, num_classes, 0].sum()) or int(host[:, num_classes, 1].sum()):
        raise CobevtHipError("seg_class_counts: labels outside [0, %d)" % num_classes)
    return host[:, :num_classes]


class DepthwisePlan(object):

    def __init__(self, weight, bn=None, stride=1, pad=(0, 0), act=0, dtype=torch.bfloat16, device="cuda"):
        w = weight.detach().double().cpu()
        c, one, kh, kw = w.shape
        if one != 1 or kh != kw:
            raise CobevtHipError("DepthwisePlan expects a (C, 1, k, k) weight")
        b = torch.zeros(c, dtype=torch.float64)
        if bn is not None:
            s_, sh = bn_affine(bn)
            w = w * s_.cpu()[:, None, None, None]
            b = sh.cpu().double()
        if c % 8 != 0:
            raise CobevtHipError("depthwise conv needs a multiple of 8 channels, got %d" % c)
        self.c, self.k, self.stride, self.act = c, kh, int(stride), int(act)
        self.pad0, self.pad1 = int(pad[0]), int(pad[1])
        self.dtype, self.code = dtype, dcode(dtype)
        self.wgt = w[:, 0].permute(1, 2, 0).reshape(kh * kw, c).to(torch.float32).to(device).contiguous()
        self.bias = b.to(torch.float32).to(device).contiguous()

    def out_hw(self, h, w):
        return ((h + self.pad0 + self.pad1 - self.k) // self.stride + 1, (w + self.pad0 + self.pad1 - self.k) // self.stride + 1)


def depthwise_conv(x, plan):
    _need_cuda(x)
    n, h, w, c = x.shape
    if c != plan.c or x.dtype != plan.dtype or not x.is_contiguous():
        raise CobevtHipError("depthwise_conv: bad input %s %s for C=%d %s" % (tuple(x.shape), x.dtype, plan.c, plan.dtype))
    ho, wo = plan.out_hw(h, w)
    out = torch.empty((n, ho, wo, c), device=x.device, dtype=plan.dtype)
    dims = _ints([plan.code, n, h, w, c, plan.k, plan.stride, plan.pad0, plan.pad0, ho, wo, plan.act])

    def cost():
        esz = 2 if plan.code == BF16 else 4
        return 2.0 * n * ho * wo * c * plan.k * plan.k, float((x.numel() + out.numel()) * esz)
# ... 136 lines not shown
```

include/cobevt_hip.h:

```cpp
#ifndef COBEVT_HIP_H
#define COBEVT_HIP_H

#include <hip/hip_runtime_api.h>

#ifdef __cplusplus
extern "C" {
#endif

#define COBEVT_OK 0
#define COBEVT_ERR_ARG 1
#define COBEVT_ERR_SHAPE 2
#define COBEVT_ERR_LAUNCH 3
#define COBEVT_ERR_UNSUPPORTED 4

int cobevt_abi_version(void);
const char* cobevt_strerror(int code);

int cobevt_conv2d_nhwc(const void* in, const void* wgt, const float* bias, const void* residual,
                       const float* pre_scale, const float* pre_shift, const int* klut, void* out,
                       const int* dims, hipStream_t stream);

int cobevt_conv3x3_nhwc(const void* in, const void* wgt, const float* bias, const void* residual, void* out,
                        const int* dims, hipStream_t stream);

// ... 17 lines not shown

int cobevt_stem_conv7x7s2_pool_u8(const unsigned char* in, const float* lut, const void* wgt, const float* bias, void* out,
                                  const int* dims, hipStream_t stream);

int cobevt_linear_rows(const void* in, const void* wgt, const float* bias, const void* residual, const float* ln_gamma,
                       const float* ln_beta, const float* pre_scale, const float* pre_shift, void* out, const long* dims,
                       float ln_eps, hipStream_t stream);

int cobevt_linear_rows_wfrag(const void* in, const void* wfrag, const float* bias, const void* residual,
                             const float* pre_scale, const float* pre_shift, void* out, const long* dims, float ln_eps,
                             hipStream_t stream);

int cobevt_attn_mlp_chain(const void* a, const void* skip, void* out, const void* wp, const float* bp, const void* w1,
                          const float* b1, const void* w2, const float* b2, const float* post_gamma,
                          const float* post_beta, const void* wnext, const float* bnext, void* out_next, const int* dims,
                          float eps1, float eps_post, float eps_next, hipStream_t stream);

int cobevt_window_attention(const void* q, const void* k, const void* v, void* out, const float* bias_table,
                            const float* mask, const int* dims, float scale, hipStream_t stream);

int cobevt_window_attention_lse(const void* q, const void* k, const void* v, void* out, float* lse, const float* bias_table,
                                const float* mask, const int* dims, float scale, float drop_p, unsigned drop_seed,
                                const unsigned* drop_seed_dev, hipStream_t stream);
int cobevt_window_attention_bwd(const void* q, const void* k, const void* v, const void* out, const float* lse,
                                const void* dout, const float* dlse, void* dq, void* dk, void* dv, float* dbias, const float* bias_table,
                                const float* mask, const int* dims, float scale, float drop_p, unsigned drop_seed,
                                const unsigned* drop_seed_dev, hipStream_t stream);
int cobevt_attention_dropout_mask(int B, int L, int heads, int Nq, int Nk, float drop_p, unsigned drop_seed, unsigned char* keep,
                                  hipStream_t stream);

int cobevt_layernorm_bwd(const float* x, const float* dy, const float* gamma, float* dx, float* dgamma, float* dbeta, int rows,
                         int C, float eps, hipStream_t stream);
int cobevt_gelu(const float* x, const float* dy, float* out, long n, hipStream_t stream);
int cobevt_layernorm_fwd_t(const void* x, const float* gamma, const float* beta, void* y, int rows, int C, float eps, const int* dtypes,
                           hipStream_t stream);
int cobevt_layernorm_bwd_t(const void* x, const void* dy, const float* gamma, void* dx, float* dgamma, float* dbeta, int rows, int C,
                           float eps, const int* dtypes, hipStream_t stream);
int cobevt_gelu_bf16(const void* x, const void* dy, void* out, long n, hipStream_t stream);
int cobevt_conv_wgrad(const void* x, const void* dy, float* dw, const int* dims, hipStream_t stream);
int cobevt_conv_wgrad_blocked(const void* xb, const void* db, float* dw, const int* dims, hipStream_t stream);

int cobevt_agent_max(const void* in, void* out, int dtype, int B, int L, long per, hipStream_t stream);

int cobevt_bottleneck_nhwc(const void* in, const void* w1, const void* w2, const void* w3, const float* b1, const float* b2,
                           const float* b3, void* out, const int* dims, hipStream_t stream);

int cobevt_bottleneck_f32_nhwc(const void* in, const void* y1, const void* w1frag, const float* b1, const void* w2frag, const float* b2,
                               const void* w3frag, const float* b3, void* out, const int* dims, hipStream_t stream);

int cobevt_attention_index_map(const int* map8, int B, int* rows, hipStream_t stream);
int cobevt_attention_bias_index(const int* qmap8, const int* kmap8, int bias_L, int* idx, hipStream_t stream);

int cobevt_layernorm(const void* in, const float* gamma, const float* beta, void* out, int dtype, int rows, int C,
                     float eps, int navg, long avg_stride, long in_batch_stride, int rows_per_batch,
                     hipStream_t stream);

int cobevt_fax_ray_embed(const float* I_inv, const float* E_inv, const float* image_plane, const float* w_img,
                         const float* w_cam, void* out, int dtype, int BN, int hw, int D, hipStream_t stream);

int cobevt_fax_bev_embed(const float* E_inv, const float* world, const float* w_bev, const float* b_bev,
                         const float* w_cam, const void* x, void* out, int dtype, int B, int n, int hw, int D,
                         int x_bcast, hipStream_t stream);

int cobevt_bev_embed_linear_rows(const float* E_inv, const float* world, const float* w_bev, const float* b_bev,
                                 const float* w_cam, const void* x, const void* wgt, const float* bias, void* out,
                                 const long* dims, float ln_eps, hipStream_t stream);

int cobevt_maxpool3x3s2(const void* in, void* out, int dtype, int N, int H, int W, int C, hipStream_t stream);

int cobevt_to_nhwc(const void* in, int in_dtype, void* out, int out_dtype, int N, int C, int H, int W,
                   const long* strides, hipStream_t stream);
int cobevt_from_nhwc(const void* in, int in_dtype, void* out, int out_dtype, int N, int C, int H, int W,
                     const long* strides, hipStream_t stream);

int cobevt_pairwise_warp(const void* x, const float* pairwise, const int* record_len, void* nb, float* roi, int dtype, int B, int L,
                         int H, int W, int C, float discrete_ratio, float downsample_rate, hipStream_t stream);
int cobevt_pairwise_warp_bwd(const void* dnb, const float* pairwise, const int* record_len, float* dx, int dtype, int B, int L, int H,
                             int W, int C, float discrete_ratio, float downsample_rate, hipStream_t stream);
int cobevt_agent_message_reduce(const void* msg, const void* ego, const float* roi, const int* record_len, void* out, int dtype,
                                int B, int L, int HW, int C, int mode, hipStream_t stream);
int cobevt_gru_zero_state(const void* in, void* out, int dtype, long rows, int C, hipStream_t stream);
int cobevt_agent_softmax_sum(const void* score, int lds, const void* nb, const float* roi, const int* record_len, void* out, int dtype,
                             int B, int L, int HW, int C, int use_mask, hipStream_t stream);

int cobevt_regroup(const void* in, const int* record_len, void* out, float* mask, int dtype, int B, int max_cav,
                   long elems_per_agent, hipStream_t stream);

int cobevt_sttf_warp(const void* x, const float* tmat, const float* cav_mask, void* out, float* com_mask,
                     const int* record_len, float* cav_out, int dtype, int B, int L, int H, int W, int C,
                     float discrete_ratio, float downsample_rate, hipStream_t stream);

int cobevt_invert_small(const float* in, float* out, int n, int dim, hipStream_t stream);

int cobevt_resize_nhwc(const void* in, void* out, int dtype, int N, int H, int W, int C, int Ho, int Wo, int mode,
                       hipStream_t stream);

int cobevt_channel_affine(const float* in, const float* scale, const float* shift, float* out, long N, int C, long HW,
                          hipStream_t stream);

int cobevt_host_fetch(const void* host_src, void* dst, long bytes, int blocks, hipStream_t stream);


int cobevt_softmax_argmax(const void* logits, float* prob, long long* map, int dtype, int N, int C, int hw,
                          hipStream_t stream);

int cobevt_seg_class_counts(const long long* pred, const long long* gt, unsigned long long* counts, int N, int hw, int K,
                            hipStream_t stream);

int cobevt_weighted_cross_entropy(const void* logits, const long long* target, const float* weight, float* scratch, float* out,
                                  int dtype, int N, int C, int hw, hipStream_t stream);
int cobevt_weighted_cross_entropy_bwd(const float* logits, const long long* target, const float* weight, const float* stats,
                                      const float* upstream, float* dlogits, int N, int C, int hw, hipStream_t stream);

int cobevt_conv3x3_head_nchw(const void* in, const float* wgt, const float* bias, float* out, int dtype, int N, int H, int W, int Cin,
                             int Cout, hipStream_t stream);

int cobevt_linear_rows_small_k(const void* in, const void* wfrag, const float* bias, const void* residual, const float* pre_scale,
                               const float* pre_shift, void* out, const long* dims, float ln_eps, hipStream_t stream);

int cobevt_bev_embed_linear_rows_small_k(const float* E_inv, const float* world, const float* w_bev, const float* b_bev,
                                         const float* w_cam, const void* x, const void* wfrag, const float* bias, void* out,
                                         const long* dims, float ln_eps, hipStream_t stream);

int cobevt_sigmoid_focal_loss(const float* pred, const float* label, const unsigned char* visibility, const unsigned int* label_mask,
                              float* scratch, float* out, int N, int C, int NL, int hw, int min_visibility, float alpha,
                              float gamma, int soft_label, hipStream_t stream);

int cobevt_iou_counts(const float* pred, const float* label, const unsigned char* visibility, const unsigned int* label_mask,
                      const float* thresholds, unsigned long long* counts, int N, int C, int NL, int hw, int T,
                      int min_visibility, hipStream_t stream);


int cobevt_depthwise_conv_nhwc(const void* in, const float* wgt, const float* bias, void* out, const int* dims,
                               hipStream_t stream);

int cobevt_spatial_mean_nhwc(const void* in, float* out, int dtype, int N, int hw, int C, hipStream_t stream);

int cobevt_se_gate(const float* mean, const float* w_reduce, const float* b_reduce, const float* w_expand,
                   const float* b_expand, float* gate, int N, int C, int Cs, hipStream_t stream);

int cobevt_channel_gate_nhwc(const void* in, const float* gate, void* out, int dtype, int N, int hw, int C,
                             hipStream_t stream);

int cobevt_mean_linear_rows_small_k(const void* in, const void* wfrag, const float* bias, void* out, const long* dims,
                                    float ln_eps, hipStream_t stream);

int cobevt_window_attention_ksplit(const void* q, const void* k, const void* v, void* out, const float* bias_table,
                                   const float* mask, void* part_out, float* part_lse, const int* dims, float scale,
                                   int ksplit, long out_rows, hipStream_t stream);

int cobevt_proj_chain(const void* a, const float* pre_scale, const float* pre_shift, const void* skip, const void* wp,
                      const float* bp, void* out, const void* wnext, const float* bnext, void* out_next, const int* dims,
                      float eps_next, hipStream_t stream);

int cobevt_proj_chain_kv(const void* a, const void* const* ptrs, const int* dims, float eps_next, hipStream_t stream);

int cobevt_swap_fusion_stage(const void* qkv, const void* x, void* out, void* qkv_next, const int* map,
                             const float* bias_table, const float* mask, const void* wp, const float* bp, const void* w1,
                             const float* b1, const void* w2, const float* b2, const void* wn, const float* bn,
                             const int* dims, float scale, float eps1, float eps_next, hipStream_t stream);


int cobevt_channel_sums(const void* x, const float* shift, double* sum, double* sumsq, float* out_f, double* scratch,
                        int scratch_blocks, int dtype, long rows, int C, hipStream_t stream);
int cobevt_f64_to_f32(const double* in, float* out, int n, hipStream_t stream);
int cobevt_bn_finalize(const double* sum, const double* sumsq, const float* gamma, const float* beta, float* running_mean,
                       float* running_var, float* scale, float* shift, float* mean, float* rstd, int C, long rows, float eps,
                       float momentum, int training, int shifted, long long* batches_tracked, hipStream_t stream);
int cobevt_bn_batch_stats(const void* x, const float* gamma, const float* beta, float* running_mean, float* running_var, float* scale,
                          float* shift, float* mean, float* rstd, double* scratch, int scratch_blocks, int dtype, long rows, int C,
                          float eps, float momentum, long long* batches_tracked, hipStream_t stream);
int cobevt_bn_apply(const void* x, const void* residual, const float* scale, const float* shift, void* y, int dtype, long rows,
                    int C, int act, hipStream_t stream);
int cobevt_bn_backward(const void* x, const void* y, const void* dy, const float* mean, const float* rstd, const float* gamma,
                       double* dgamma_dbeta, float* grads_f, double* scratch, int scratch_blocks, void* dx, void* dres, int dtype,
                       long rows, int C, int act, int training, hipStream_t stream);
int cobevt_maxpool3x3s2_bwd(const void* x, const void* dy, float* dx, int dtype, int N, int H, int W, int C, hipStream_t stream);
int cobevt_fax_bev_query_train(const float* grid, const float* w, const float* bias, const float* c, const float* x, float* out,
                               const int* dims, hipStream_t stream);
int cobevt_fax_bev_query_train_bwd(const float* grid, const float* w, const float* bias, const float* c, const float* dq, float* dx,
                                   float* dw, float* dbias, float* dc, const int* dims, hipStream_t stream);
int cobevt_group_mean(const void* in, void* out, int dtype, long B, int n, long inner, int backward, hipStream_t stream);
int cobevt_maxpool3x3s2_bwd_t(const void* x, const void* dy, void* dx, int dtype, int N, int H, int W, int C, hipStream_t stream);
int cobevt_pixel_unshuffle2_nhwc(const void* in, void* out, int dtype, int N, int Ho, int Wo, int C, int inverse,
                                 hipStream_t stream);
int cobevt_upsample_nearest2_nhwc(const void* in, void* out, int dtype, int N, int H, int W, int C, int backward,
                                  hipStream_t stream);
int cobevt_sttf_warp_bwd(const float* dout, const float* tmat, const int* record_len, float* dx, int B, int L, int H, int W, int C,
                         float discrete_ratio, float downsample_rate, hipStream_t stream);

int cobevt_conv_weight_rows(const float* w, void* rows_fwd, void* rows_dgrad, const int* dims, hipStream_t stream);
int cobevt_conv3_weight_operands(const float* w, void* frag, void* rows3, const int* dims, hipStream_t stream);
int cobevt_conv3_weight_operands2(const float* w, void* const* outs, const int* dims, hipStream_t stream);
int cobevt_linear_weight_frags(const float* w, void* frag, void* frag_t, const int* dims, hipStream_t stream);
int cobevt_conv_wgrad3_chunks(const int* dims);
int cobevt_conv_wgrad3(const void* x, const void* dy, float* dw, float* scratch, const int* dims, hipStream_t stream);
int cobevt_linear_wgrad_chunks(const long* dims);
int cobevt_linear_wgrad(const void* x, const void* dy, float* dw, float* scratch, const long* dims, hipStream_t stream);
int cobevt_wgrad_block_operand(const void* src, void* dst, const int* dims, hipStream_t stream);

int cobevt_swish(const void* x, const void* dy, void* out, int dtype, long n, hipStream_t stream);
int cobevt_depthwise_wgrad(const void* x, const void* dy, float* dw, const int* dims, hipStream_t stream);
int cobevt_resize_bilinear_bwd(const void* dy, float* dx, int dtype, int N, int H, int W, int C, int Ho, int Wo, hipStream_t stream);
int cobevt_sigmoid_focal_loss_bwd(const float* pred, const float* label, const unsigned char* visibility, const unsigned int* label_mask,
                                  const float* stats, const float* gscale, float* dpred, int N, int C, int NL, int hw, int min_visibility,
                                  float alpha, float gamma, int soft_label, hipStream_t stream);


int cobevt_peer_window_alloc(long bytes, void** dptr, void* handle64);
int cobevt_peer_window_open(const void* handle64, void** dptr);
int cobevt_peer_window_close(void* dptr);
int cobevt_peer_window_free(void* dptr);
int cobevt_peer_window_status(const void* window, long bytes, int* status, int* epoch, hipStream_t stream);
int cobevt_peer_window_status_async(const void* window, long bytes, unsigned int* host_words, hipStream_t stream);
int cobevt_peer_exchange(const void* local, void* const* windows, int world, int rank, int n_local, long block_bytes,
                         const int* dest_rank, const int* dest_block, long window_bytes, long spin_limit,
                         hipStream_t stream);

int cobevt_calibrate_mfma(float* out, long long* clk, int blocks, int iters, hipStream_t stream);
int cobevt_calibrate_copy(const void* src, void* dst, long bytes, hipStream_t stream);
int cobevt_calibrate_clock_khz(int* wall_khz, int* sclk_max_khz);

int cobevt_pillar_vfe(const float* voxel_features, const int* voxel_num_points, const int* voxel_coords, const float* w,
                      const float* shift, const int* record_len, void* out, float* cav_mask, const int* dims, const float* geom,
                      hipStream_t stream);
int cobevt_scatter_rows(const void* rows, const int* voxel_coords, void* out, int dtype, long P, int C, int N, int ny, int nx,
                        hipStream_t stream);

int cobevt_pillar_train_scratch(long P, long* stats_doubles, long* bwd_floats);
int cobevt_pillar_train_stats(const float* voxel_features, const int* voxel_num_points, const int* voxel_coords, const int* record_len,
                              const float* w, const float* gamma, const float* beta, float* running_mean, float* running_var,
                              long* num_batches_tracked, int* order, long* dst, int* count, double* partial, float* w_folded,
                              float* shift_folded, double* stat, const int* dims, const float* geom, int mode, float eps, float momentum,
                              hipStream_t stream);
int cobevt_pillar_train_bwd(const float* voxel_features, const int* voxel_num_points, const int* voxel_coords, const int* order,
                            const long* dst, const int* count, const float* w_folded, const float* shift_folded, const float* w,
                            const float* gamma, const double* stat, const float* dout, float* partial, float* dw, float* dgamma,
                            float* dbeta, const int* dims, const float* geom, int mode, hipStream_t stream);
int cobevt_gather_rows(const void* canvas, const int* voxel_coords, void* rows, int dtype, long P, int C, int N, int ny, int nx,
                       hipStream_t stream);

int cobevt_voxelize_scratch(const long* dims, long* workspace_ints);
int cobevt_voxelize_points(const float* points, const int* point_offsets, float* voxel_features, int* voxel_coords,
                           int* voxel_num_points, int* num_voxels, int* workspace, const long* dims, const float* geom,
                           hipStream_t stream);

int cobevt_detect_scratch(long total_anchors, long* workspace_bytes);
int cobevt_detect_post(const float* const* psm, const float* const* rm, const float* const* anchors, const float* matrices,
                       const int* cav_dims, int ncav, int hwl, float score_threshold, float nms_thresh, float* boxes, float* scores,
                       int* index, int* count, void* workspace, hipStream_t stream);
int cobevt_nms_rotated(const float* box_corners, const float* box_scores, long N, int corner_floats, float nms_thresh, float* boxes,
                       float* scores, int* index, int* count, void* workspace, hipStream_t stream);
int cobevt_delta_to_boxes3d(const float* rm, const float* anchors, float* boxes3d, int N, int H, int W, int A, hipStream_t stream);
int cobevt_rotated_iou(const float* a, const float* b, double* iou, long N, long M, hipStream_t stream);

#ifdef __cplusplus
}
#endif
#endif
```

Measured before the change: 615.1.

## Fuse ray embedding into the proj_chain128 kernel and add row prefetch

The kernel now computes the camera-ray embedding per row and uses it as the skip/residual term, so the key projection no longer needs a separate ray_embed kernel and its global write and read. Per-camera intrinsics, extrinsics, cam terms and w_img are staged in LDS. The change also specialises the skip modes at compile time, prefetches the next row block's activations when each wave handles several blocks, replaces double-buffered weight tiles with per-fragment reloads interleaved with the MFMAs, and makes the wave count a tunable. In exchange it uses more LDS and registers, and the setup cost per block grows with the number of cameras.

```diff
diff --git a/cobevt_amd/csrc/elementwise.hip b/cobevt_amd/csrc/elementwise.hip
--- a/cobevt_amd/csrc/elementwise.hip
+++ b/cobevt_amd/csrc/elementwise.hip
@@ -1,3 +1,4 @@
+#include "ray_embed.hpp"
 #include "warp_common.hpp"
 #include "wave_ops.hpp"
 
@@ -62,7 +63,7 @@
         const int ch = gl * 8 + e;
         const float4 a = *(const float4*)(w_img + ch * 4), c = *(const float4*)(w_cam + ch * 4);
         wi[e][0] = a.x; wi[e][1] = a.y; wi[e][2] = a.z; wi[e][3] = a.w;
-        ce[e] = c.x * E[3] + c.y * E[7] + c.z * E[11] + c.w * E[15];
+        ce[e] = ray_cam_term(c, E);
     }
     const int p0 = blockIdx.x * kRayPixPerBlock;
     constexpr int U = 4;
@@ -78,23 +79,16 @@
         const int pix = pb + u * ngroups;
         if (pix >= min(p0 + kRayPixPerBlock, hw)) break;
         const float px = pxs[u], py = pys[u], pz = pzs[u];
-        float cam[4];
-#pragma unroll
-        for (int r = 0; r < 3; ++r) cam[r] = I[r * 3 + 0] * px + I[r * 3 + 1] * py + I[r * 3 + 2] * pz;
-        cam[3] = 1.f;
         float d4[4];
-#pragma unroll
-        for (int r = 0; r < 4; ++r)
-            d4[r] = E[r * 4 + 0] * cam[0] + E[r * 4 + 1] * cam[1] + E[r * 4 + 2] * cam[2] + E[r * 4 + 3] * cam[3];
+        ray_direction(I, E, px, py, pz, d4);
         float v[8], ss = 0.f;
 #pragma unroll
         for (int e = 0; e < 8; ++e) {
-            const float de = wi[e][0] * d4[0] + wi[e][1] * d4[1] + wi[e][2] * d4[2] + wi[e][3] * d4[3];
-            v[e] = de - ce[e];
+            v[e] = ray_channel(make_float4(wi[e][0], wi[e][1], wi[e][2], wi[e][3]), d4, ce[e]);
             ss += v[e] * v[e];
         }
         ss = wave_sum_xor(ss, G);
-        const float inv = 1.0f / (sqrtf(ss) + 1e-7f);
+        const float inv = ray_inv_norm(ss);
 #pragma unroll
         for (int e = 0; e < 8; ++e) v[e] *= inv;
         store8<T>(out + ((size_t)bn * hw + pix) * D + gl * 8, v);
diff --git a/cobevt_amd/csrc/proj_chain128.hip b/cobevt_amd/csrc/proj_chain128.hip
--- a/cobevt_amd/csrc/proj_chain128.hip
+++ b/cobevt_amd/csrc/proj_chain128.hip
@@ -1,3 +1,4 @@
+#include "ray_embed.hpp"
 #include "row_chain.hpp"
 #include "wave_ops.hpp"
 
@@ -10,22 +11,68 @@
 constexpr int kSc = 0, kSh = 128, kBp = 256, kBn = 384;
 constexpr int kTabFloats = 640;
 constexpr int kLdsBytes = kTab + kTabFloats * 4;
-
-template <int NNT, int NW>
-__global__ __launch_bounds__(NW * 64, 1) void proj_chain128_kernel(RowChainParams p, int nblk) {
+constexpr int kRayWi = kTabFloats, kRayCam = kRayWi + 512, kRayCamStride = 160, kRayI = 128, kRayE = 140;
+constexpr int kMaxCams = 64;
+constexpr int ray_lds_bytes(int cams) { return kLdsBytes + (512 + cams * kRayCamStride) * 4; }
+constexpr int kMinWaves = 8, kMaxWaves = 12;
+
+template <int NNT, int MAXW, int SKIP, bool PF>
+__global__ __launch_bounds__(MAXW * 64, 1) void proj_chain128_kernel(RowChainParams p, RayEmbedParams ray, int nblk) {
     extern __shared__ __attribute__((aligned(16))) unsigned char smem[];
     const uint4* wl = (const uint4*)smem;
     float* tab = (float*)(smem + kTab);
     const int tid = threadIdx.x, lane = tid & 63, wave = tid >> 6;
     const int h = lane >> 5, ql = lane & 31;
-
+    const int nthreads = blockDim.x, nw = nthreads >> 6;
+    constexpr bool EMB = SKIP == 2;
+
+    auto load_rows = [&](uint4 (&r)[8], float (&px)[3], int blk) {
+        const int m = blk * 32 + ql;
+        const size_t grow = (blk < nblk && m < p.M) ? m : p.M - 1;
+        const bf16_t* arow = p.a + grow * 128;
+#pragma unroll
+        for (int g = 0; g < 8; ++g) r[g] = *(const uint4*)(arow + 16 * g + 8 * h);
+        if constexpr (EMB) {
+            const int pix = (int)(grow % (size_t)ray.hw);
+#pragma unroll
+            for (int e = 0; e < 3; ++e) px[e] = ray.plane[(size_t)e * ray.hw + pix];
+        }
+    };
+    int blk = blockIdx.x * nw + wave;
+    uint4 af[8];
+    float apx[3] = {0.f, 0.f, 0.f};
+    load_rows(af, apx, blk);
+
+    if constexpr (EMB) {
+        const int nce = ray.BN * 128;
+        for (int i0 = tid; i0 < nce; i0 += 4 * nthreads) {
+            float ce[4];
+#pragma unroll
+            for (int u = 0; u < 4; ++u) {
+                const int i = min(i0 + u * nthreads, nce - 1);
+                ce[u] = ray_cam_term(*(const float4*)(ray.w_cam + (i & 127) * 4), ray.E_inv + (i >> 7) * 16);
+            }
+#pragma unroll
+            for (int u = 0; u < 4; ++u) {
+                const int i = i0 + u * nthreads;
+                if (i < nce) tab[kRayCam + (i >> 7) * kRayCamStride + (i & 127)] = ce[u];
+            }
+        }
+        for (int i = tid; i < ray.BN * 32; i += nthreads) {
+            const int c = i >> 5, e = i & 31;
+            if (e < 9) tab[kRayCam + c * kRayCamStride + kRayI + e] = ray.I_inv[c * 9 + e];
+            else if (e >= 12 && e < 28) tab[kRayCam + c * kRayCamStride + kRayE + e - 12] = ray.E_inv[c * 16 + e - 12];
+        }
+        for (int i = tid; i < 512; i += nthreads) tab[kRayWi + i] = ray.w_img[i];
+    }
     {
         uint4* dst = (uint4*)smem;
-        constexpr int TOTAL = (kFn + NNT * 8) * 64, PER = (TOTAL + NW * 64 - 1) / (NW * 64);
+        constexpr int MINW = MAXW == 8 ? 8 : 9;
+        constexpr int TOTAL = (kFn + NNT * 8) * 64, PER = (TOTAL + MINW * 64 - 1) / (MINW * 64);
         uint4 tmp[PER];
 #pragma unroll
         for (int u = 0; u < PER; ++u) {
-            const int i = tid + u * NW * 64, ic = i < TOTAL ? i : TOTAL - 1;
+            const int i = tid + u * nthreads, ic = i < TOTAL ? i : TOTAL - 1;
             const int f = ic >> 6, ln = ic & 63, hh = ln >> 5, q = ln & 31;
             const uint4* base = f < kFn ? p.wp + (size_t)f * 64 : p.wn + (size_t)(f - kFn) * 64;
             const unsigned char* a0 = (const unsigned char*)(base + (f < kFn ? ln : q)) + (f < kFn ? 0 : 8 * hh);
@@ -35,10 +82,10 @@
         }
 #pragma unroll
         for (int u = 0; u < PER; ++u) {
-            const int i = tid + u * NW * 64;
+            const int i = tid + u * nthreads;
             if (i < TOTAL) dst[i] = tmp[u];
         }
-        for (int i = tid; i < kTabFloats; i += NW * 64) {
+        for (int i = tid; i < kTabFloats; i += nthreads) {
             float v;
             if (i < kSh) v = p.pre_scale ? p.pre_scale[i] : 1.f;
             else if (i < kBp) v = p.pre_shift ? p.pre_shift[i - kSh] : 0.f;
@@ -55,24 +102,26 @@
 #pragma unroll
         for (int g = 0; g < 8; ++g) fr[g] = wl[(first + g) * 64 + lane + opq];
     };
-    const int nwaves = gridDim.x * NW;
-    for (int blk = blockIdx.x * NW + wave; blk < nblk; blk += nwaves) {
+    auto load_frag = [&](uint4& f, int idx) { f = wl[idx * 64 + lane + opq]; };
+    const int nwaves = gridDim.x * nw;
+    for (; blk < nblk; blk += nwaves) {
         asm volatile("" : "+v"(opq));
         const int m0 = blk * 32;
         const bool live = m0 + ql < p.M;
         const size_t grow = live ? m0 + ql : p.M - 1;
-        const bf16_t* arow = p.a + grow * 128;
-        uint4 af[8], sk[8];
-#pragma unroll
-        for (int g = 0; g < 8; ++g) af[g] = *(const uint4*)(arow + 16 * g + 8 * h);
-        if (p.skip) {
+        uint4 sk[SKIP == 1 ? 8 : 1];
+        if constexpr (SKIP == 1) {
             const bf16_t* srow = p.skip + (size_t)(grow % p.skip_rows) * 128;
 #pragma unroll
             for (int g = 0; g < 8; ++g) sk[g] = *(const uint4*)(srow + 16 * g + 8 * h);
-        } else {
-#pragma unroll
-            for (int g = 0; g < 8; ++g) sk[g] = make_uint4(0, 0, 0, 0);
-        }
+        }
+        uint4 nx[PF ? 8 : 1];
+        float npx[3] = {0.f, 0.f, 0.f};
+        const bool more = PF && blk + nwaves < nblk;
+        if constexpr (PF) {
+            if (more) load_rows(nx, npx, blk + nwaves);
+        }
+
 #pragma unroll
         for (int g = 0; g < 8; ++g) {
             float v[8];
@@ -88,28 +137,64 @@
         }
 
         float y[4][16];
-        uint4 fr[2][8];
-        load_tile(fr[0], kFp);
+        uint2 ek[EMB ? 16 : 1];
+        if constexpr (EMB) {
+            const int cam = (int)(grow / (size_t)ray.hw);
+            const float* ct = tab + kRayCam + cam * kRayCamStride + opq;
+            float d4[4];
+            ray_direction(ct + kRayI, ct + kRayE, apx[0], apx[1], apx[2], d4);
+            float ss = 0.f, einv = 0.f;
+#pragma unroll
+            for (int pass = 0; pass < 2; ++pass) {
+#pragma unroll
+                for (int tk = 0; tk < 16; ++tk) {
+                    const int ch = 8 * tk + 4 * h;
+                    const float4 ce = *(const float4*)(ct + ch);
+                    const float4* wi = (const float4*)(tab + kRayWi + opq) + ch;
+                    const float v0 = ray_channel(wi[0], d4, ce.x), v1 = ray_channel(wi[1], d4, ce.y);
+                    const float v2 = ray_channel(wi[2], d4, ce.z), v3 = ray_channel(wi[3], d4, ce.w);
+                    if (pass == 0) { ss += v0 * v0; ss += v1 * v1; ss += v2 * v2; ss += v3 * v3; }
+                    else ek[tk] = make_uint2(ray_store_bf16x2(v0, v1, einv), ray_store_bf16x2(v2, v3, einv));
+                    if (tk & 1) __builtin_amdgcn_sched_barrier(0);
+                }
+                if (pass == 0) einv = ray_inv_norm(xhalf_sum(ss));
+            }
+        }
+        uint4 fr[8];
+        load_tile(fr, kFp);
 #pragma unroll
         for (int t = 0; t < 4; ++t) {
             f32x16 acc;
 #pragma unroll
             for (int r = 0; r < 16; ++r) acc[r] = 0.f;
-            load_tile(fr[(t + 1) & 1], t < 3 ? kFp + (t + 1) * 8 : kFn);
             __builtin_amdgcn_sched_barrier(0);
 #pragma unroll
-            for (int g = 0; g < 8; ++g) mfma_kgroup<bf16_t>(fr[t & 1][g], af[g], acc);
+            for (int g = 0; g < 8; ++g) {
+                mfma_kgroup<bf16_t>(fr[g], af[g], acc);
+                load_frag(fr[g], 8 * (t + 1) + g);
+            }
 #pragma unroll
             for (int m = 0; m < 2; ++m) {
-                uint2 s0 = make_uint2(sk[2 * t + m].x, sk[2 * t + m].y), s1 = make_uint2(sk[2 * t + m].z, sk[2 * t + m].w);
-                half_swap(s0, s1);
                 const float4 b0 = *(const float4*)(tab + kBp + 32 * t + 16 * m + 4 * h + opq);
                 const float4 b1 = *(const float4*)(tab + kBp + 32 * t + 16 * m + 8 + 4 * h + opq);
                 float* d = &y[t][8 * m];
-                d[0] = rbf(acc[8 * m + 0] + b0.x + bf2f(s0.x & 0xffff)); d[1] = rbf(acc[8 * m + 1] + b0.y + bf2f(s0.x >> 16));
-                d[2] = rbf(acc[8 * m + 2] + b0.z + bf2f(s0.y & 0xffff)); d[3] = rbf(acc[8 * m + 3] + b0.w + bf2f(s0.y >> 16));
-                d[4] = rbf(acc[8 * m + 4] + b1.x + bf2f(s1.x & 0xffff)); d[5] = rbf(acc[8 * m + 5] + b1.y + bf2f(s1.x >> 16));
-                d[6] = rbf(acc[8 * m + 6] + b1.z + bf2f(s1.y & 0xffff)); d[7] = rbf(acc[8 * m + 7] + b1.w + bf2f(s1.y >> 16));
+                if constexpr (EMB) {
+                    const uint2 e0 = ek[4 * t + 2 * m], e1 = ek[4 * t + 2 * m + 1];
+                    d[0] = rbf(acc[8 * m + 0] + b0.x + bf2f(e0.x & 0xffff)); d[1] = rbf(acc[8 * m + 1] + b0.y + bf2f(e0.x >> 16));
+                    d[2] = rbf(acc[8 * m + 2] + b0.z + bf2f(e0.y & 0xffff)); d[3] = rbf(acc[8 * m + 3] + b0.w + bf2f(e0.y >> 16));
+                    d[4] = rbf(acc[8 * m + 4] + b1.x + bf2f(e1.x & 0xffff)); d[5] = rbf(acc[8 * m + 5] + b1.y + bf2f(e1.x >> 16));
+                    d[6] = rbf(acc[8 * m + 6] + b1.z + bf2f(e1.y & 0xffff)); d[7] = rbf(acc[8 * m + 7] + b1.w + bf2f(e1.y >> 16));
+                } else if constexpr (SKIP == 0) {
+                    d[0] = rbf(acc[8 * m + 0] + b0.x); d[1] = rbf(acc[8 * m + 1] + b0.y); d[2] = rbf(acc[8 * m + 2] + b0.z); d[3] = rbf(acc[8 * m + 3] + b0.w);
+                    d[4] = rbf(acc[8 * m + 4] + b1.x); d[5] = rbf(acc[8 * m + 5] + b1.y); d[6] = rbf(acc[8 * m + 6] + b1.z); d[7] = rbf(acc[8 * m + 7] + b1.w);
+                } else {
+                    uint2 s0 = make_uint2(sk[2 * t + m].x, sk[2 * t + m].y), s1 = make_uint2(sk[2 * t + m].z, sk[2 * t + m].w);
+                    half_swap(s0, s1);
+                    d[0] = rbf(acc[8 * m + 0] + b0.x + bf2f(s0.x & 0xffff)); d[1] = rbf(acc[8 * m + 1] + b0.y + bf2f(s0.x >> 16));
+                    d[2] = rbf(acc[8 * m + 2] + b0.z + bf2f(s0.y & 0xffff)); d[3] = rbf(acc[8 * m + 3] + b0.w + bf2f(s0.y >> 16));
+                    d[4] = rbf(acc[8 * m + 4] + b1.x + bf2f(s1.x & 0xffff)); d[5] = rbf(acc[8 * m + 5] + b1.y + bf2f(s1.x >> 16));
+                    d[6] = rbf(acc[8 * m + 6] + b1.z + bf2f(s1.y & 0xffff)); d[7] = rbf(acc[8 * m + 7] + b1.w + bf2f(s1.y >> 16));
+                }
             }
         }
         if (p.out) {
@@ -152,10 +237,12 @@
             f32x16 acc;
 #pragma unroll
             for (int r = 0; r < 16; ++r) acc[r] = 0.f;
-            if (n + 1 < NNT) load_tile(fr[(n + 1) & 1], kFn + (n + 1) * 8);
             __builtin_amdgcn_sched_barrier(0);
 #pragma unroll
-            for (int g = 0; g < 8; ++g) mfma_kgroup<bf16_t>(fr[n & 1][g], yh[g], acc);
+            for (int g = 0; g < 8; ++g) {
+                mfma_kgroup<bf16_t>(fr[g], yh[g], acc);
+                if (n + 1 < NNT) load_frag(fr[g], kFn + 8 * (n + 1) + g);
+            }
             float nv[16];
 #pragma unroll
             for (int k = 0; k < 4; ++k) {
@@ -171,27 +258,52 @@
                 if (live) *(uint4*)(nrow + 32 * n + 16 * m + 8 * h) = make_uint4(r0.x, r0.y, r1.x, r1.y);
             }
         }
-    }
-}
-
-template <int NNT> int launch128(const RowChainParams& p, hipStream_t stream) {
-    constexpr int NW = 8;
-    cobevt::allow_dynamic_lds<proj_chain128_kernel<NNT, NW>>(kLdsBytes);
+        if constexpr (PF) {
+            if (more) {
+#pragma unroll
+                for (int g = 0; g < 8; ++g) af[g] = nx[g];
+#pragma unroll
+                for (int e = 0; e < 3; ++e) apx[e] = npx[e];
+            }
+        }
+    }
+}
+
+template <int NNT, int MAXW, int SKIP, bool PF> int launch_as(const RowChainParams& p, const RayEmbedParams& ray, int nw, int nblk, hipStream_t stream) {
+    cobevt::allow_dynamic_lds<proj_chain128_kernel<NNT, MAXW, SKIP, PF>>(SKIP == 2 ? ray_lds_bytes(kMaxCams) : kLdsBytes);
+    int blocks = (nblk + nw - 1) / nw;
+    if (blocks > 256) blocks = 256;
+    hipLaunchKernelGGL((proj_chain128_kernel<NNT, MAXW, SKIP, PF>), dim3((unsigned)blocks), dim3(nw * 64), SKIP == 2 ? ray_lds_bytes(ray.BN) : kLdsBytes,
+                       stream, p, ray, nblk);
+    return cobevt::launch_status();
+}
+
+template <int NNT, int SKIP> int launch128(const RowChainParams& p, const RayEmbedParams& ray, int nw, hipStream_t stream) {
     const int nblk = (p.M + 31) / 32;
-    int blocks = (nblk + NW - 1) / NW;
-    if (blocks > 256) blocks = 256;
-    hipLaunchKernelGGL((proj_chain128_kernel<NNT, NW>), dim3((unsigned)blocks), dim3(NW * 64), kLdsBytes, stream, p, nblk);
-    return cobevt::launch_status();
-}
-
-}
-
-int launch_proj_chain128(const RowChainParams& p, hipStream_t stream) {
+    if (nw == 0) nw = kMinWaves;
+    const bool pf = nblk > 256 * nw;
+    if (nw <= 8) return pf ? launch_as<NNT, 8, SKIP, true>(p, ray, nw, nblk, stream) : launch_as<NNT, 8, SKIP, false>(p, ray, nw, nblk, stream);
+    return pf ? launch_as<NNT, 12, SKIP, true>(p, ray, nw, nblk, stream) : launch_as<NNT, 12, SKIP, false>(p, ray, nw, nblk, stream);
+}
+
+}
+
+int launch_proj_chain128(const RowChainParams& p, const RayEmbedParams* ray, int nw, hipStream_t stream) {
     if (p.C != 128 || !p.wn || !p.out_next || p.Nn % 32 != 0 || p.Nn > 32 * kMaxNnt || p.next_act != 0) return -1;
     if (p.M < 32768) return -1;
+    if (nw != 0 && (nw < kMinWaves || nw > kMaxWaves)) return -1;
+    if (ray) {
+        if (p.skip || ray->BN < 1 || ray->BN > kMaxCams || ray->hw < 1 || (long)ray->BN * ray->hw != (long)p.M) return -1;
+        switch (p.Nn / 32) {
+            case 4: return launch128<4, 2>(p, *ray, nw, stream);
+            case 8: return launch128<8, 2>(p, *ray, nw, stream);
+            default: return -1;
+        }
+    }
+    const RayEmbedParams none = {nullptr, nullptr, nullptr, nullptr, nullptr, 0, 0};
     switch (p.Nn / 32) {
-        case 4: return launch128<4>(p, stream);
-        case 8: return launch128<8>(p, stream);
+        case 4: return p.skip ? launch128<4, 1>(p, none, nw, stream) : launch128<4, 0>(p, none, nw, stream);
+        case 8: return p.skip ? launch128<8, 1>(p, none, nw, stream) : launch128<8, 0>(p, none, nw, stream);
         default: return -1;
     }
 }
diff --git a/cobevt_amd/csrc/ray_embed.hpp b/cobevt_amd/csrc/ray_embed.hpp
--- /dev/null
+++ b/cobevt_amd/csrc/ray_embed.hpp
@@ -0,0 +1,36 @@
+#pragma once
+#include "common.hpp"
+
+namespace cobevt {
+
+struct RayEmbedParams {
+    const float* I_inv;
+    const float* E_inv;
+    const float* plane;
+    const float* w_img;
+    const float* w_cam;
+    int BN, hw;
+};
+
+__device__ __forceinline__ void ray_direction(const float* I, const float* E, float px, float py, float pz, float (&d4)[4]) {
+    float cam[4];
+#pragma unroll
+    for (int r = 0; r < 3; ++r) cam[r] = I[r * 3 + 0] * px + I[r * 3 + 1] * py + I[r * 3 + 2] * pz;
+    cam[3] = 1.f;
+#pragma unroll
+    for (int r = 0; r < 4; ++r)
+        d4[r] = E[r * 4 + 0] * cam[0] + E[r * 4 + 1] * cam[1] + E[r * 4 + 2] * cam[2] + E[r * 4 + 3] * cam[3];
+}
+
+__device__ __forceinline__ float ray_cam_term(float4 c, const float* E) { return c.x * E[3] + c.y * E[7] + c.z * E[11] + c.w * E[15]; }
+
+__device__ __forceinline__ float ray_channel(float4 w, const float (&d4)[4], float ce) {
+    const float de = w.x * d4[0] + w.y * d4[1] + w.z * d4[2] + w.w * d4[3];
+    return de - ce;
+}
+
+__device__ __forceinline__ float ray_inv_norm(float ss) { return 1.0f / (sqrtf(ss) + 1e-7f); }
+
+__device__ __forceinline__ uint32_t ray_store_bf16x2(float v0, float v1, float inv) { return pack_bf2(v0 * inv, v1 * inv); }
+
+}
diff --git a/cobevt_amd/csrc/row_chain.hip b/cobevt_amd/csrc/row_chain.hip
--- a/cobevt_amd/csrc/row_chain.hip
+++ b/cobevt_amd/csrc/row_chain.hip
@@ -1,3 +1,4 @@
+#include "ray_embed.hpp"
 #include "row_chain.hpp"
 #include "wave_ops.hpp"
 
@@ -338,13 +339,11 @@
     return cobevt::launch_status();
 }
 
-extern "C" int cobevt_proj_chain(const void* a, const float* pre_scale, const float* pre_shift, const void* skip, const void* wp,
-                                 const float* bp, void* out, const void* wnext, const float* bnext, void* out_next, const int* dims,
-                                 float eps_next, hipStream_t stream) {
+static int proj_chain_params(RowChainParams& p, const void* a, const float* pre_scale, const float* pre_shift, const void* skip, const void* wp,
+                             const float* bp, void* out, const void* wnext, const float* bnext, void* out_next, const int* dims, float eps_next) {
     if (!a || !wp || !wnext || !bnext || !out_next || !dims) return COBEVT_ERR_ARG;
     if ((pre_scale == nullptr) != (pre_shift == nullptr)) return COBEVT_ERR_ARG;
     if (dims[0] != 0) return COBEVT_ERR_UNSUPPORTED;
-    RowChainParams p;
     p.a = (const bf16_t*)a; p.skip = (const bf16_t*)skip; p.out = (bf16_t*)out;
     p.wp = (const uint4*)wp; p.bp = bp;
     p.w1 = (const uint4*)wnext; p.b1 = bnext; p.w2 = (const uint4*)wnext; p.b2 = bnext;
@@ -358,10 +357,40 @@
     if (p.M < 1 || p.C != 128) return COBEVT_ERR_SHAPE;
     if (p.Nn < 8 || p.Nn % 8 || p.Nn > kRcBnMax || p.next_act < 0 || p.next_act > 2) return COBEVT_ERR_SHAPE;
     if (p.skip_rows > p.M || p.M % p.skip_rows) return COBEVT_ERR_SHAPE;
-    if (dims[8] == 0) {
-        const int rc = launch_proj_chain128(p, stream);
+    if (dims[8] != 0 && dims[8] != 1 && (dims[8] < 8 || dims[8] > 12)) return COBEVT_ERR_ARG;
+    return COBEVT_OK;
+}
+
+extern "C" int cobevt_proj_chain(const void* a, const float* pre_scale, const float* pre_shift, const void* skip, const void* wp,
+                                 const float* bp, void* out, const void* wnext, const float* bnext, void* out_next, const int* dims,
+                                 float eps_next, hipStream_t stream) {
+    RowChainParams p;
+    const int st = proj_chain_params(p, a, pre_scale, pre_shift, skip, wp, bp, out, wnext, bnext, out_next, dims, eps_next);
+    if (st != COBEVT_OK) return st;
+    if (dims[8] != 1) {
+        const int rc = launch_proj_chain128(p, nullptr, dims[8], stream);
         if (rc >= 0) return rc;
     }
     launch_chain<1, 32, true, false>(p, stream);
     return cobevt::launch_status();
 }
+
+extern "C" int cobevt_proj_chain_ray(const void* a, const float* pre_scale, const float* pre_shift, const void* const* ray, const void* wp,
+                                     const float* bp, void* out, const void* wnext, const float* bnext, void* out_next, const int* dims,
+                                     float eps_next, hipStream_t stream) {
+    if (!ray || !dims) return COBEVT_ERR_ARG;
+    for (int i = 0; i < 5; ++i)
+        if (!ray[i]) return COBEVT_ERR_ARG;
+    const int hw = dims[6], cams = dims[9];
+    if (hw < 1 || cams < 1 || (long)hw * cams != (long)dims[1]) return COBEVT_ERR_SHAPE;
+    int d[9];
+    for (int i = 0; i < 9; ++i) d[i] = dims[i];
+    d[6] = 0;
+    RowChainParams p;
+    const int st = proj_chain_params(p, a, pre_scale, pre_shift, nullptr, wp, bp, out, wnext, bnext, out_next, d, eps_next);
+    if (st != COBEVT_OK) return st;
+    if (d[8] == 1) return COBEVT_ERR_UNSUPPORTED;
+    const RayEmbedParams rp = {(const float*)ray[0], (const float*)ray[1], (const float*)ray[2], (const float*)ray[3], (const float*)ray[4], cams, hw};
+    const int rc = launch_proj_chain128(p, &rp, d[8], stream);
+    return rc >= 0 ? rc : COBEVT_ERR_UNSUPPORTED;
+}
diff --git a/cobevt_amd/csrc/row_chain.hpp b/cobevt_amd/csrc/row_chain.hpp
--- a/cobevt_amd/csrc/row_chain.hpp
+++ b/cobevt_amd/csrc/row_chain.hpp
@@ -27,7 +27,8 @@
 };
 
 int launch_row_chain64(const RowChainParams& p, hipStream_t stream);
-int launch_proj_chain128(const RowChainParams& p, hipStream_t stream);
+struct RayEmbedParams;
+int launch_proj_chain128(const RowChainParams& p, const RayEmbedParams* ray, int nw, hipStream_t stream);
 
 int launch_row_chain_f32(const void* a, const void* skip, void* out, const void* wp, const float* bp, const void* w1, const float* b1,
                          const void* w2, const float* b2, const float* post_g, const float* post_b, const void* wnext, const float* bnext,
diff --git a/cobevt_amd/host/fax_modules.py b/cobevt_amd/host/fax_modules.py
--- a/cobevt_amd/host/fax_modules.py
+++ b/cobevt_amd/host/fax_modules.py
@@ -248,7 +248,13 @@
         plane = rt.f32_param(self, "plane", self.image_plane, (3, h * w))
         w_img = rt.f32_param(self, "w_img", self.img_embed.weight, (d, 4))
         w_cam = rt.f32_param(self, "w_cam", self.cam_embed.weight, (d, 4))
-        img = ops.ray_embed(I_inv, E_inv, plane, w_img, w_cam, h * w, d, dt).reshape(bn, h, w, d)
+
+        def ray_map():
+            return ops.ray_embed(I_inv, E_inv, plane, w_img, w_cam, h * w, d, dt).reshape(bn, h, w, d)
+
+        ray_in_kernel = (not padded and self.feature_proj is not None and dt == torch.bfloat16 and d == 128 and feature.shape[-1] == 128
+                         and ops.proj_chain_ray_fusable(bn * h * w, bn))
+        img = None if ray_in_kernel else ray_map()
 
         def kv_buffer(tag):
             if not padded:
@@ -260,6 +266,12 @@
         pk, pv = self._pair_plan("k"), self._pair_plan("v")
         plan_key = rt.conv_plan(self, "fproj", self.feature_proj[2], pre_bn=self.feature_proj[0]) if self.feature_proj is not None else None
         plan_val = rt.conv_plan(self, "flin", self.feature_linear[2], pre_bn=self.feature_linear[0])
+        if ray_in_kernel:
+            if ops.proj_chain_fusable(feature, plan_key, pk, None) and ops.proj_chain_fusable(feature, plan_val, pv, None):
+                kk = ops.proj_chain(feature, plan_key, pk, ray=(I_inv, E_inv, plane, w_img, w_cam, h * w), out_next=o.get("kk"))
+                vv = ops.proj_chain(feature, plan_val, pv, out_next=o.get("vv"))
+                return {"n": n, "hp": hp, "wp": wp, "kk": kk, "vv": vv}
+            img = ray_map()
         if (not padded and plan_key is not None and ops.proj_chain_fusable(feature, plan_key, pk, img)
                 and ops.proj_chain_fusable(feature, plan_val, pv, None)):
             kk = ops.proj_chain(feature, plan_key, pk, residual=img, out_next=o.get("kk"))
diff --git a/cobevt_amd/lib.py b/cobevt_amd/lib.py
--- a/cobevt_amd/lib.py
+++ b/cobevt_amd/lib.py
@@ -85,6 +85,7 @@
     "cobevt_se_gate": (ctypes.c_int, [_vp, _vp, _vp, _vp, _vp, _vp, ctypes.c_int, ctypes.c_int, ctypes.c_int, _vp]),
     "cobevt_mean_linear_rows_small_k": (ctypes.c_int, [_vp, _vp, _vp, _vp, _c_long_p, ctypes.c_float, _vp]),
     "cobevt_proj_chain": (ctypes.c_int, [_vp] * 10 + [_c_int_p, ctypes.c_float, _vp]),
+    "cobevt_proj_chain_ray": (ctypes.c_int, [_vp] * 3 + [ctypes.POINTER(ctypes.c_void_p)] + [_vp] * 6 + [_c_int_p, ctypes.c_float, _vp]),
     "cobevt_proj_chain_kv": (ctypes.c_int, [_vp, ctypes.POINTER(ctypes.c_void_p), _c_int_p, ctypes.c_float, _vp]),
     "cobevt_swap_fusion_stage": (ctypes.c_int, [_vp, _vp, _vp, _vp, _c_int_p, _vp, _vp, _vp, _vp, _vp, _vp, _vp, _vp, _vp, _vp, _c_int_p,
                                                 ctypes.c_float, ctypes.c_float, ctypes.c_float, _vp]),
diff --git a/cobevt_amd/ops.py b/cobevt_amd/ops.py
--- a/cobevt_amd/ops.py
+++ b/cobevt_amd/ops.py
@@ -41,6 +41,9 @@
 USE_PROJ_CHAIN = True
 USE_PROJ_CHAIN_KV = True
 USE_PROJ_CHAIN_WAVE = True
+USE_PROJ_CHAIN_RAY = True
+PROJ_CHAIN_WAVES = 0
+PROJ_CHAIN_RAY_MIN_ROWS, PROJ_CHAIN_RAY_MAX_CAMS = 32768, 64
 USE_SWAP_STAGE = True
 USE_BOTTLENECK = True
 ATTN_VARIANT = 0
@@ -49,7 +52,7 @@
 ATTN_QSPLIT = 0
 
 INT_KNOBS = ("CONV3_VARIANT", "BASICBLOCK_TILE_ROWS", "ROW_CHAIN_ROWS", "GEMM_ROWS3_MIN_M", "GEMM_ROWS3_MAX_K", "GEMM_ROWS3_STRIDED",
-             "GEMM_ROWS3_ROWS64_MIN_M", "BASICBLOCK_MAX_C", "ATTN_VARIANT", "ATTN_QSPLIT", "ATTN_KSPLIT")
+             "GEMM_ROWS3_ROWS64_MIN_M", "BASICBLOCK_MAX_C", "ATTN_VARIANT", "ATTN_QSPLIT", "ATTN_KSPLIT", "PROJ_CHAIN_WAVES")
 
 
 def dcode(dtype):
@@ -769,8 +772,9 @@
     _need_cuda(i_inv, e_inv, image_plane, w_img, w_cam)
     bn = i_inv.shape[0]
     out = torch.empty((bn, hw, dim), device=i_inv.device, dtype=dtype)
-    _L.call("cobevt_fax_ray_embed", _p(i_inv), _p(e_inv), _p(image_plane), _p(w_img), _p(w_cam), _p(out), dcode(dtype), bn, hw, dim,
-            _stream())
+    with _timed("ray_embed|D%d M=%d" % (dim, bn * hw), lambda: (0.0, float(out.numel() * out.element_size()))):
+        _L.call("cobevt_fax_ray_embed", _p(i_inv), _p(e_inv), _p(image_plane), _p(w_img), _p(w_cam), _p(out), dcode(dtype), bn, hw, dim,
+                _stream())
     return out
 
 
@@ -1388,23 +1392,60 @@
             and (residual is None or (residual.is_contiguous() and residual.shape == x.shape and residual.dtype == x.dtype)))
 
 
-def proj_chain(x, plan_p, next_plan, residual=None, out_next=None):
-    _need_cuda(x, residual)
+def _ray_check(ray, m, c):
+    if len(ray) != 6:
+        raise CobevtHipError("proj_chain: `ray` is (I_inv, E_inv, image_plane, w_img, w_cam, hw)")
+    i_inv, e_inv, plane, w_img, w_cam, hw = ray
+    bn = i_inv.shape[0]
+    for name, t, numel in (("I_inv", i_inv, bn * 9), ("E_inv", e_inv, bn * 16), ("image_plane", plane, 3 * hw), ("w_img", w_img, c * 4),
+                           ("w_cam", w_cam, c * 4)):
+        if t.dtype != torch.float32 or not t.is_contiguous() or t.numel() != numel:
+            raise CobevtHipError("proj_chain: ray embedding operand %s must be a contiguous fp32 tensor of %d elements (got %s, %s%s)"
+                                 % (name, numel, tuple(t.shape), t.dtype, "" if t.is_contiguous() else ", not contiguous"))
+    if bn * hw != m:
+        raise CobevtHipError("proj_chain: %d cameras x %d pixels != %d rows" % (bn, hw, m))
+    return bn
+
+
+def proj_chain_ray_fusable(m, cams):
+    return (USE_PROJ_CHAIN_RAY and USE_PROJ_CHAIN_WAVE and m >= PROJ_CHAIN_RAY_MIN_ROWS and cams <= PROJ_CHAIN_RAY_MAX_CAMS)
+
+
+def proj_chain(x, plan_p, next_plan, residual=None, out_next=None, ray=None, out=None):
+    _need_cuda(x, residual, out)
     c, nn_ = 128, next_plan.cout
     m = x.numel() // c
     if out_next is None:
         out_next = torch.empty(x.shape[:-1] + (nn_,), device=x.device, dtype=x.dtype)
     elif out_next.numel() != m * nn_ or not out_next.is_contiguous() or out_next.dtype != x.dtype:
         raise CobevtHipError("proj_chain: `out_next` must be a contiguous (.., %d) buffer of dtype %s" % (nn_, x.dtype))
-    dims = _ints([0, m, c, nn_, int(next_plan.has_ln), next_plan.act, 0, plan_p.pre_relu, 0 if USE_PROJ_CHAIN_WAVE else 1])
+    if out is not None and (out.numel() != m * c or not out.is_contiguous() or out.dtype != x.dtype):
+        raise CobevtHipError("proj_chain: `out` must be a contiguous (.., %d) buffer of dtype %s" % (c, x.dtype))
+    variant = (PROJ_CHAIN_WAVES or 0) if USE_PROJ_CHAIN_WAVE else 1
+    in_kernel = False
+    if ray is not None:
+        if residual is not None:
+            raise CobevtHipError("proj_chain: `ray` and `residual` are two spellings of the same operand")
+        _need_cuda(*ray[:5])
+        cams = _ray_check(ray, m, c)
+        in_kernel = proj_chain_ray_fusable(m, cams)
+        if not in_kernel:
+            residual = ray_embed(*ray[:5], ray[5], c, x.dtype).reshape(x.shape)
 
     def cost():
         return 2.0 * m * (c * c + c * nn_), float(m * (c * (2 if residual is not None else 1) + nn_) * 2 + (c * c + c * nn_) * 2)
 
-    with _timed("row_chain|proj C%d M=%d +next%d" % (c, m, nn_), cost):
-        _L.call("cobevt_proj_chain", _p(x), _p(plan_p.pre_scale), _p(plan_p.pre_shift), _p(residual), _p(plan_p.wfrag_rows),
-                _p(plan_p.bias), None, _p(next_plan.wfrag_rows), _p(next_plan.bias), _p(out_next), dims, ctypes.c_float(next_plan.ln_eps),
-                _stream())
+    with _timed("row_chain|proj C%d M=%d +next%d%s" % (c, m, nn_, " ray" if in_kernel else ""), cost):
+        if in_kernel:
+            ptrs = (ctypes.c_void_p * 5)(*[t.data_ptr() for t in ray[:5]])
+            dims = _ints([0, m, c, nn_, int(next_plan.has_ln), next_plan.act, ray[5], plan_p.pre_relu, variant, cams])
+            _L.call("cobevt_proj_chain_ray", _p(x), _p(plan_p.pre_scale), _p(plan_p.pre_shift), ptrs, _p(plan_p.wfrag_rows), _p(plan_p.bias),
+                    _p(out), _p(next_plan.wfrag_rows), _p(next_plan.bias), _p(out_next), dims, ctypes.c_float(next_plan.ln_eps), _stream())
+        else:
+            dims = _ints([0, m, c, nn_, int(next_plan.has_ln), next_plan.act, 0, plan_p.pre_relu, variant])
+            _L.call("cobevt_proj_chain", _p(x), _p(plan_p.pre_scale), _p(plan_p.pre_shift), _p(residual), _p(plan_p.wfrag_rows),
+                    _p(plan_p.bias), _p(out), _p(next_plan.wfrag_rows), _p(next_plan.bias), _p(out_next), dims, ctypes.c_float(next_plan.ln_eps),
+                    _stream())
     return out_next
 
 
diff --git a/include/cobevt_hip.h b/include/cobevt_hip.h
--- a/include/cobevt_hip.h
+++ b/include/cobevt_hip.h
@@ -193,6 +193,10 @@
 int cobevt_proj_chain(const void* a, const float* pre_scale, const float* pre_shift, const void* skip, const void* wp,
                       const float* bp, void* out, const void* wnext, const float* bnext, void* out_next, const int* dims,
                       float eps_next, hipStream_t stream);
+
+int cobevt_proj_chain_ray(const void* a, const float* pre_scale, const float* pre_shift, const void* const* ray, const void* wp,
+                          const float* bp, void* out, const void* wnext, const float* bnext, void* out_next, const int* dims,
+                          float eps_next, hipStream_t stream);
 
 int cobevt_proj_chain_kv(const void* a, const void* const* ptrs, const int* dims, float eps_next, hipStream_t stream);
 
```

New measurement: 616.2 (median of 3 runs). About the same (+0.2%).
